# modelscope/FunASR

Hardware: AMD Instinct MI355X
Metric: audio-seconds/sec (RTF^-1) Paraformer-large 30s@bs64 (higher is better)
Workload: dtype f32 (GEMM / self-attention operands split into 2 fp16 planes, 3 fp16 MFMA products, f32 accumulate; all else f32)

## Files before the change

### funasr_amd/csrc/gemm_f16x2.hip

```cpp
#include "common.h"
#include <cstdlib>
#include <type_traits>
#include "gemm_f16x2_epilogue.h"

namespace pf {

namespace {

typedef _Float16 f16x8 __attribute__((ext_vector_type(8)));

template <int WM, int WN, int WGM = 4, int KS_ = 32> struct Geo2 {
    static constexpr int NW = WGM * 2;
    static constexpr int BM = WGM * WM * 32, BN = 2 * WN * 32;
    static constexpr int KS = KS_, ROWB = 2 * KS, CPR = ROWB / 16, RPP = 1024 / ROWB;
    static constexpr int SWZ = CPR == 4 ? 2 : 3;
    static constexpr int A_PLANE_B = BM * ROWB, B_PLANE_B = BN * ROWB;
    static constexpr int STAGE_B = 2 * (A_PLANE_B + B_PLANE_B);
    static constexpr int NSTG = KS == 16 ? (WGM == 4 ? (163840 / STAGE_B > 6 ? 6 : 163840 / STAGE_B) : 3) : 2;
    static constexpr int NPIECE = STAGE_B / 1024;
    static constexpr int A_PIECES = 2 * BM / RPP;
    static constexpr int PPW = NPIECE / NW;
    static constexpr int ELD = WN * 32 + 4;
    static constexpr int SLAB_B = NW * 32 * ELD * 4;
    static constexpr int LDS_B = NSTG * STAGE_B > SLAB_B ? NSTG * STAGE_B : SLAB_B;
};
template <int N> __device__ __forceinline__ void glds_wait_but() { asm volatile("s_waitcnt vmcnt(%0)" ::"i"(N) : "memory"); }

template <int WM, int WN, int MODE, int OUT, int ABL, int SCHED, int WGM, int KS_>
__device__ __forceinline__ void gemm2_tile_body(Gemm2Args& p, const int m0, const int n0, const int nblk, unsigned char* smem) {
    typedef Geo2<WM, WN, WGM, KS_> G;
    constexpr int BM = G::BM, BN = G::BN, KS = G::KS, ROWB = G::ROWB, CPR = G::CPR, RPP = G::RPP, PPW = G::PPW;
    constexpr int STAGE_B = G::STAGE_B, A_PLANE_B = G::A_PLANE_B, B_PLANE_B = G::B_PLANE_B;
    const int tid = threadIdx.x;
    const int lane = tid & 63;
    const int wave = __builtin_amdgcn_readfirstlane(tid >> 6);
    const int wr = wave >> 1, wc = wave & 1;
    const int hh = lane >> 5, idx = lane & 31;

    const unsigned short* src[PPW];
    {
        const int prow = lane / CPR;
        const int chunk = (lane % CPR) ^ ((prow >> G::SWZ) & (CPR - 1));
#pragma unroll
        for (int i = 0; i < PPW; ++i) {
            const int q = wave + G::NW * i;
            if (q < G::A_PIECES) {
                int row = m0 + (q % (BM / RPP)) * RPP + prow;
                row = row < p.M ? row : p.M - 1;
                src[i] = p.A + (size_t)(q / (BM / RPP)) * p.a_plane + (size_t)row * p.lda + chunk * 8;
            } else {
                const int qq = q - G::A_PIECES;
                int col = n0 + (qq % (BN / RPP)) * RPP + prow;
                col = col < p.N ? col : p.N - 1;
                src[i] = p.W + (size_t)(qq / (BN / RPP)) * p.w_plane + (size_t)col * p.ldw + chunk * 8;
            }
        }
    }
    const unsigned lds0 = __builtin_amdgcn_readfirstlane(lds_addr_of(smem) + (unsigned)wave * 1024);
    const size_t a_step = p.a_kstep > 0 ? (size_t)p.a_kstep : (size_t)KS, w_step = p.w_kstep > 0 ? (size_t)p.w_kstep : (size_t)KS;
    auto piece = [&](int i, int buf, int kt) {
        if constexpr (ABL == 3) return;
        glds16(src[i] + kt * (i < G::A_PIECES / G::NW ? a_step : w_step), lds0 + (unsigned)buf * STAGE_B + (unsigned)i * (G::NW * 1024));
    };

    floatx16 acc[WM][WN];
#pragma unroll
    for (int i = 0; i < WM; ++i)
#pragma unroll
        for (int jj = 0; jj < WN; ++jj)
#pragma unroll
            for (int r = 0; r < 16; ++r) acc[i][jj][r] = 0.f;

    const int f = (idx >> G::SWZ) & (CPR - 1);
    const int aoff = (wr * (WM * 32) + idx) * ROWB;
    const int boff = 2 * A_PLANE_B + (wc * (WN * 32) + idx) * ROWB;
    int coff[2];
#pragma unroll
    for (int st = 0; st < 2; ++st) coff[st] = ((2 * st + hh) ^ f) * 16;

    const int nk = p.K / KS;
    if constexpr (SCHED == 3) { if (wave >= 4) __builtin_amdgcn_s_setprio(1); }
    if constexpr (KS_ == 16 && WGM == 4) {
        constexpr int R = G::NSTG;
        static_assert(R == 5 && G::NPIECE == 32 && G::A_PIECES == 16 && RPP == 32, "deep ring: five 32-KB stages of 32-row pieces");
        const int grp = wave >> 1, hw = wave & 1;
        const int prow = lane / CPR;
        const unsigned chunkb = (unsigned)(((lane % CPR) ^ ((prow >> G::SWZ) & (CPR - 1))) * 16);
        const unsigned ldsb = __builtin_amdgcn_readfirstlane(lds_addr_of(smem));
        const size_t a_step2 = (p.a_kstep > 0 ? (size_t)p.a_kstep : (size_t)KS) * 2, w_step2 = (p.w_kstep > 0 ? (size_t)p.w_kstep : (size_t)KS) * 2;
        auto issue = [&](int kt, int buf, int i) {
            if constexpr (ABL == 3) return;
            const unsigned dst = ldsb + (unsigned)buf * STAGE_B + (unsigned)(hw + 2 * i) * 1024;
            if (i < 8) {
                int row = m0 + (hw + 2 * (i & 3)) * RPP + prow;
                row = row < p.M ? row : p.M - 1;
                glds16s(reinterpret_cast<const char*>(p.A) + (size_t)(i >> 2) * p.a_plane * 2 + (size_t)kt * a_step2,
                        (unsigned)row * (unsigned)p.lda * 2u + chunkb, dst);
            } else {
                int col = n0 + (hw + 2 * (i & 3)) * RPP + prow;
                col = col < p.N ? col : p.N - 1;
                glds16s(reinterpret_cast<const char*>(p.W) + (size_t)((i - 8) >> 2) * p.w_plane * 2 + (size_t)kt * w_step2,
                        (unsigned)col * (unsigned)p.ldw * 2u + chunkb, dst);
            }
        };
        auto issue_stage = [&](int kt, int buf) {
#pragma unroll
            for (int i = 0; i < 16; ++i) issue(kt, buf, i);
        };
        auto frags = [&](f16x8 (&a)[WM][2], f16x8 (&b)[WN][2], int buf) {
            const unsigned char* sb = smem + buf * STAGE_B;
#pragma unroll
            for (int pl = 1; pl >= 0; --pl) {
#pragma unroll
                for (int i = 0; i < WM; ++i)
                    a[i][pl] = __builtin_bit_cast(f16x8, *reinterpret_cast<const uint4*>(sb + pl * A_PLANE_B + aoff + i * 32 * ROWB + coff[0]));
            }
#pragma unroll
            for (int pl = 0; pl < 2; ++pl) {
#pragma unroll
                for (int jj = 0; jj < WN; ++jj)
                    b[jj][pl] = __builtin_bit_cast(f16x8, *reinterpret_cast<const uint4*>(sb + pl * B_PLANE_B + boff + jj * 32 * ROWB + coff[0]));
            }
        };
        if (grp < nk) issue_stage(grp, grp);
        if (grp == 0) glds_wait_all();
        __syncthreads();
        if (grp == 0 && 4 < nk) issue_stage(4, 4);
        f16x8 a0[WM][2], b0[WN][2], a1[WM][2], b1[WN][2];
        frags(a0, b0, 0);
        int buf = 0;
        auto step = [&](auto more, int kt, f16x8 (&a)[WM][2], f16x8 (&b)[WN][2], f16x8 (&an)[WM][2], f16x8 (&bn)[WN][2]) {
            const int nbuf = buf + 1 == R ? 0 : buf + 1;
            if constexpr (decltype(more)::value) {
                const bool own = grp == ((kt + 1) & 3);
                asm volatile("s_waitcnt lgkmcnt(0)" ::: "memory");
                if (own) glds_wait_all();
                __syncthreads();
                frags(an, bn, nbuf);
                if (own && kt + R < nk) issue_stage(kt + R, buf);
                __builtin_amdgcn_sched_barrier(0);
            }
#pragma unroll
            for (int i = 0; i < WM; ++i)
#pragma unroll
                for (int jj = 0; jj < WN; ++jj) acc[i][jj] = __builtin_amdgcn_mfma_f32_32x32x16_f16(a[i][1], b[jj][0], acc[i][jj], 0, 0, 0);
#pragma unroll
            for (int i = 0; i < WM; ++i)
#pragma unroll
                for (int jj = 0; jj < WN; ++jj) acc[i][jj] = __builtin_amdgcn_mfma_f32_32x32x16_f16(a[i][0], b[jj][1], acc[i][jj], 0, 0, 0);
#pragma unroll
            for (int i = 0; i < WM; ++i)
#pragma unroll
                for (int jj = 0; jj < WN; ++jj) acc[i][jj] = __builtin_amdgcn_mfma_f32_32x32x16_f16(a[i][0], b[jj][0], acc[i][jj], 0, 0, 0);
            buf = nbuf;
        };
        typedef std::integral_constant<bool, true> More;
        typedef std::integral_constant<bool, false> Last;
        for (int kt = 0; kt + 2 < nk; kt += 2) {
            step(More{}, kt, a0, b0, a1, b1);
            step(More{}, kt + 1, a1, b1, a0, b0);
        }
        step(More{}, nk - 2, a0, b0, a1, b1);
        step(Last{}, nk - 1, a1, b1, a0, b0);
    } else if constexpr (KS_ == 16) {
#pragma unroll
        for (int i = 0; i < PPW; ++i) piece(i, 0, 0);
        if (nk > 1) {
#pragma unroll
            for (int i = 0; i < PPW; ++i) piece(i, 1, 1);
        }
        for (int kt = 0; kt < nk; ++kt) {
            if (kt + 1 < nk) glds_wait_but<PPW>(); else glds_wait_all();
            __syncthreads();
            const unsigned char* sb = smem + (kt % 3) * STAGE_B;
            f16x8 a[WM][2], b[WN][2];
#pragma unroll
            for (int pl = 0; pl < 2; ++pl) {
#pragma unroll
                for (int i = 0; i < WM; ++i)
                    a[i][pl] = __builtin_bit_cast(f16x8, *reinterpret_cast<const uint4*>(sb + pl * A_PLANE_B + aoff + i * 32 * ROWB + coff[0]));
#pragma unroll
                for (int jj = 0; jj < WN; ++jj)
                    b[jj][pl] = __builtin_bit_cast(f16x8, *reinterpret_cast<const uint4*>(sb + pl * B_PLANE_B + boff + jj * 32 * ROWB + coff[0]));
            }
            if (kt + 2 < nk) {
#pragma unroll
                for (int i = 0; i < PPW; ++i) piece(i, (kt + 2) % 3, kt + 2);
            }
#define PF_PROD16(PA, PB)                                                                                             \
    _Pragma("unroll") for (int i = 0; i < WM; ++i) _Pragma("unroll") for (int jj = 0; jj < WN; ++jj)                  \
        acc[i][jj] = __builtin_amdgcn_mfma_f32_32x32x16_f16(a[i][PA], b[jj][PB], acc[i][jj], 0, 0, 0)
            PF_PROD16(1, 0);
            PF_PROD16(0, 1);
            PF_PROD16(0, 0);
#undef PF_PROD16
        }
    } else {
#pragma unroll
    for (int i = 0; i < PPW; ++i) piece(i, 0, 0);
    for (int kt = 0; kt < nk; ++kt) {
        glds_wait_all();
        __syncthreads();
        const bool nxt = kt + 1 < nk;
        const int nb = (kt + 1) & 1;
        const unsigned char* sb = smem + (kt & 1) * STAGE_B;
#define PF_PIECE(I) do { if ((I) < PPW && nxt) piece((I) < PPW ? (I) : 0, nb, kt + 1); } while (0)
#define PF_PROD(PA, PB)                                                                                               \
    _Pragma("unroll") for (int i = 0; i < WM; ++i) _Pragma("unroll") for (int jj = 0; jj < WN; ++jj)                  \
        acc[i][jj] = __builtin_amdgcn_mfma_f32_32x32x16_f16(a[i][PA], b[jj][PB], acc[i][jj], 0, 0, 0)
#define PF_LOAD(S)                                                                                                    \
    _Pragma("unroll") for (int pl = 0; pl < 2; ++pl) {                                                                \
        _Pragma("unroll") for (int i = 0; i < WM; ++i)                                                                \
            a[i][pl] = __builtin_bit_cast(f16x8, *reinterpret_cast<const uint4*>(sb + pl * A_PLANE_B + aoff + i * 32 * ROWB + coff[S]));   \
        _Pragma("unroll") for (int jj = 0; jj < WN; ++jj)                                                             \
            b[jj][pl] = __builtin_bit_cast(f16x8, *reinterpret_cast<const uint4*>(sb + pl * B_PLANE_B + boff + jj * 32 * ROWB + coff[S])); \
    }
        if constexpr (SCHED == 0 || SCHED == 3) {
            f16x8 a[WM][2], b[WN][2];
            PF_LOAD(0)
            PF_PROD(1, 0); PF_PIECE(0); PF_PIECE(1);
            PF_PROD(0, 1); PF_PIECE(2); PF_PIECE(3);
            PF_PROD(0, 0); PF_PIECE(4);
            PF_LOAD(1)
            PF_PROD(1, 0); PF_PIECE(5); PF_PIECE(6);
            PF_PROD(0, 1); PF_PIECE(7);
            PF_PROD(0, 0);
        } else {
            f16x8 a[WM][2], b[WN][2], a1[WM][2], b1[WN][2];
            PF_LOAD(0)
            {
#define a a1
#define b b1
                PF_LOAD(1)
#undef a
#undef b
            }
            if constexpr (SCHED == 2) { PF_PIECE(0); PF_PIECE(1); PF_PIECE(2); PF_PIECE(3); }
            PF_PROD(1, 0); if constexpr (SCHED == 1) { PF_PIECE(0); PF_PIECE(1); } else { PF_PIECE(4); PF_PIECE(5); }
            PF_PROD(0, 1); if constexpr (SCHED == 1) { PF_PIECE(2); PF_PIECE(3); } else { PF_PIECE(6); PF_PIECE(7); }
            PF_PROD(0, 0); if constexpr (SCHED == 1) { PF_PIECE(4); }
#define a a1
#define b b1
            PF_PROD(1, 0); if constexpr (SCHED == 1) { PF_PIECE(5); PF_PIECE(6); }
            PF_PROD(0, 1); if constexpr (SCHED == 1) { PF_PIECE(7); }
            PF_PROD(0, 0);
#undef a
#undef b
        }
#undef PF_PROD
#undef PF_LOAD
#undef PF_PIECE
    }
    }

    gemm2_epilogue<WM, WN, G::NW, MODE, OUT, ABL>(p, acc, smem, m0, n0, nblk, wave, wr, wc, lane);
}
template <int WM, int WN, int MODE, int OUT, int ABL = 0, int SCHED = 0, int WGM = 4, int KS_ = 32>
__global__ __launch_bounds__(WGM * 128, 2) void gemm_f16x2_kernel(Gemm2Args p, int nM, int nN) {
    typedef Geo2<WM, WN, WGM, KS_> G;
    constexpr int BM = G::BM, BN = G::BN;
    extern __shared__ __attribute__((aligned(16))) unsigned char smem[];

    const int L = blockIdx.x;
    const int xcd = L & 7, j8 = L >> 3;
    const int mblk = (j8 / nN) * 8 + xcd, nblk = j8 % nN;
    if (mblk >= nM) return;
    const int m0 = mblk * BM, n0 = nblk * BN;
    if constexpr (OUT == 0 && MODE == 0) {
        if (p.kslices > 1) {
            const size_t z = blockIdx.y;
            p.A += z * (size_t)p.K;
            p.W += z * (size_t)p.K;
            p.C += z * (size_t)p.M * (size_t)p.ldc;
        }
    }

    gemm2_tile_body<WM, WN, MODE, OUT, ABL, SCHED, WGM, KS_>(p, m0, n0, nblk, smem);
}


__global__ __launch_bounds__(256) void split2_kernel(const float* __restrict__ x, int ldx, unsigned short* __restrict__ y,
                                                     int ldy, size_t plane, int M, int N, float scale,
                                                     const float* __restrict__ scale_dev, int seq_out, int seq_in) {
    if (scale_dev) scale *= *scale_dev;
    const int c4n = ldy >> 2;
    const size_t total = (size_t)M * c4n;
    const bool wide_st = ldy % 8 == 0 && plane % 8 == 0 && ((uintptr_t)y & 15) == 0;
    for (size_t i = (size_t)blockIdx.x * 256 + threadIdx.x; i < total; i += (size_t)gridDim.x * 256) {
        const int row = (int)(i / c4n), c = (int)(i % c4n) * 4;
        int xrow = row;
        bool pad = false;
        if (seq_out > 0) {
            const int b = row / seq_out, t = row % seq_out;
            pad = t >= seq_in;
            xrow = b * seq_in + t;
        }
        float v[4] = {0.f, 0.f, 0.f, 0.f};
        if (pad) {
        } else if (c + 3 < N) {
            const float4 t = *reinterpret_cast<const float4*>(x + (size_t)xrow * ldx + c);
            v[0] = t.x; v[1] = t.y; v[2] = t.z; v[3] = t.w;
        } else {
#pragma unroll
            for (int e = 0; e < 4; ++e) if (c + e < N) v[e] = x[(size_t)xrow * ldx + c + e];
        }
        if (wide_st) store_split2x4_pair(y + (size_t)row * ldy + c, plane, v, scale, threadIdx.x);
        else store_split2x4(y + (size_t)row * ldy + c, plane, v, scale);
    }
}

__global__ __launch_bounds__(256) void absmax_kernel(const float* __restrict__ x, size_t n, unsigned* __restrict__ out) {
    float m = 0.f;
    for (size_t i = (size_t)blockIdx.x * 256 + threadIdx.x; i < n; i += (size_t)gridDim.x * 256) m = fmaxf(m, fabsf(x[i]));
    m = wave_max(m);
    if ((threadIdx.x & 63) == 0) atomicMax(out, __builtin_bit_cast(unsigned, m));
}

__global__ __launch_bounds__(256) void rowl1_bound_kernel(const float* __restrict__ W, int rows, int cols, int ld,
                                                          const float* __restrict__ bias, float in_bound, unsigned* __restrict__ out) {
    const int row = blockIdx.x * 4 + (threadIdx.x >> 6), lane = threadIdx.x & 63;
    if (row >= rows) return;
    float a = 0.f;
    for (int k = lane; k < cols; k += 64) a += fabsf(W[(size_t)row * ld + k]);
    a = wave_sum(a);
    const float bnd = (in_bound * a) * 1.0001f + (bias ? fabsf(bias[row]) : 0.f);
    if (lane == 0) atomicMax(out, __builtin_bit_cast(unsigned, bnd));
}

__global__ __launch_bounds__(256) void splitk_reduce_kernel(const float* __restrict__ part, int slices, size_t slice_stride, int M, int N,
                                                            const float* __restrict__ bias, int relu, const float* R1, int ldr1,
                                                            const float* R2, int ldr2, float* C, int ldc, unsigned short* C2, int ldc2,
                                                            size_t c_plane, float cscale) {
    const int n4 = N >> 2;
    const size_t total = (size_t)M * n4;
    for (size_t i = (size_t)blockIdx.x * 256 + threadIdx.x; i < total; i += (size_t)gridDim.x * 256) {
        const int row = (int)(i / n4), col = (int)(i % n4) * 4;
        const float* src = part + (size_t)row * N + col;
        float4 v = *reinterpret_cast<const float4*>(src);
        for (int z = 1; z < slices; ++z) {
            const float4 t = *reinterpret_cast<const float4*>(src + (size_t)z * slice_stride);
            v.x += t.x; v.y += t.y; v.z += t.z; v.w += t.w;
        }
        if (bias) {
            const float4 b = *reinterpret_cast<const float4*>(bias + col);
            v.x += b.x; v.y += b.y; v.z += b.z; v.w += b.w;
        }
        if (relu) { v.x = fmaxf(v.x, 0.f); v.y = fmaxf(v.y, 0.f); v.z = fmaxf(v.z, 0.f); v.w = fmaxf(v.w, 0.f); }
        if (R1) {
            const float4 r = *reinterpret_cast<const float4*>(R1 + (size_t)row * ldr1 + col);
            v.x = v.x + r.x; v.y = v.y + r.y; v.z = v.z + r.z; v.w = v.w + r.w;
        }
        if (R2) {
            const float4 r = *reinterpret_cast<const float4*>(R2 + (size_t)row * ldr2 + col);
            v.x = r.x + v.x; v.y = r.y + v.y; v.z = r.z + v.z; v.w = r.w + v.w;
        }
        if (C2) {
            const float o[4] = {v.x, v.y, v.z, v.w};
            store_split2x4(C2 + (size_t)row * ldc2 + col, c_plane, o, cscale);
        } else {
            *reinterpret_cast<float4*>(C + (size_t)row * ldc + col) = v;
        }
    }
}

template <int WM, int WN, int MODE, int OUT, int ABL = 0, int SCHED = 0, int WGM = 4, int KS_ = 32>
int launch_tile(const Gemm2Args& a, hipStream_t stream) {
    typedef Geo2<WM, WN, WGM, KS_> G;
    static PerDeviceOnce configured;
    if (!configured.done()) {
        PF_HIP_TRY(hipFuncSetAttribute(reinterpret_cast<const void*>(&gemm_f16x2_kernel<WM, WN, MODE, OUT, ABL, SCHED, WGM, KS_>),
                                       hipFuncAttributeMaxDynamicSharedMemorySize, G::LDS_B));
        configured.mark();
    }
    const int nM = ceil_div(a.M, G::BM), nN = ceil_div(a.N, G::BN);
    const int nMpad = (nM + 7) / 8 * 8;
    const unsigned gy = (OUT == 0 && MODE == 0 && a.kslices > 1) ? (unsigned)a.kslices : 1u;
    hipLaunchKernelGGL((gemm_f16x2_kernel<WM, WN, MODE, OUT, ABL, SCHED, WGM, KS_>), dim3((unsigned)nMpad * nN, gy), dim3(WGM * 128), G::LDS_B, stream, a, nM, nN);
    PF_HIP_TRY(hipGetLastError());
    return 0;
}
#if defined(PF_MEASUREMENT_KERNELS)
template <int MODE, int OUT>
int launch_pair(const Gemm2Args& a, hipStream_t stream) { return launch_tile<2, 4, MODE, OUT, 0, 0, 2, 16>(a, stream); }
template <int MODE, int OUT>
int launch_ring(const Gemm2Args& a, hipStream_t stream) { return launch_tile<2, 4, MODE, OUT, 0, 0, 4, 16>(a, stream); }
#endif
template <int MODE, int OUT>
int launch_one(const Gemm2Args& a, hipStream_t stream) {
    if constexpr (OUT == 1) {
        if (a.tile == 3) return launch_tile<2, 2, MODE, 1, 0, 0, 2>(a, stream);
    }
    if constexpr (OUT == 0) {
        if (a.tile == 3) return launch_tile<2, 2, MODE, 0, 0, 0, 2>(a, stream);
    }
#if defined(PF_MEASUREMENT_KERNELS)
    if constexpr (OUT == 0) {
        if (a.tile >= 256) return (a.tile >> 8) == 1 ? launch_tile<2, 4, MODE, 0, 0, 1>(a, stream) : launch_tile<2, 4, MODE, 0, 0, 2>(a, stream);
    }
    if constexpr (MODE == 0 && OUT == 0) {
        if (a.tile == 0x82) return launch_tile<2, 2, 0, 0, 2, 0, 2>(a, stream);
        if (a.tile == 0x83) return launch_tile<2, 2, 0, 0, 3, 0, 2>(a, stream);
        if (a.tile >= 16) {
            switch (a.tile >> 4) {
                case 1: return launch_tile<2, 4, 0, 0, 1>(a, stream);
                case 2: return launch_tile<2, 4, 0, 0, 2>(a, stream);
                case 3: return launch_tile<2, 4, 0, 0, 3>(a, stream);
                default: return launch_tile<2, 4, 0, 0, 4>(a, stream);
            }
        }
    }
#endif
    const int n_cu = device_cu_count();
    const long m_tiles = ceil_div(a.M, 256);
    const long wide_blocks = m_tiles * (a.N / 256), narrow_blocks = m_tiles * ceil_div(a.N, 128);
    const double cost_wide = (double)((wide_blocks + n_cu - 1) / n_cu), cost_narrow = 0.57 * (double)((narrow_blocks + n_cu - 1) / n_cu);
    const bool wide = a.tile == 2 || a.tile == 8 || a.tile == 9 || (a.tile == 0 && a.N % 256 == 0 && cost_wide <= cost_narrow);
    if constexpr (OUT == 0) {
        const long small_blocks = (long)ceil_div(a.M, 128) * ceil_div(a.N, 128);
        const double cost_small = 0.55 * (double)((small_blocks + 2 * n_cu - 1) / (2 * n_cu));
        if (a.tile == 0 && cost_small < (wide ? cost_wide : cost_narrow)) return launch_tile<2, 2, MODE, 0, 0, 0, 2>(a, stream);
    }
    if constexpr (OUT == 1) {
        if (a.tile == 0 && 2 * narrow_blocks <= n_cu) return launch_tile<2, 2, MODE, 1, 0, 0, 2>(a, stream);
    }
#if defined(PF_MEASUREMENT_KERNELS)
    if (wide && a.tile == 8) return launch_tile<2, 4, MODE, OUT, 0, 2>(a, stream);
    if (wide && a.tile == 9) return launch_tile<2, 4, MODE, OUT, 0, 3>(a, stream);
#endif
    return wide ? launch_tile<2, 4, MODE, OUT, 0, 0>(a, stream) : launch_tile<2, 2, MODE, OUT>(a, stream);
}

}

__global__ void pow2_scale_kernel(const float* __restrict__ amax, float* __restrict__ sc) {
    const float a = *amax;
    int e = a > 0.f ? (int)floorf(log2f(32768.f / a)) : 0;
    e = e > 100 ? 100 : (e < -100 ? -100 : e);
    sc[0] = ldexpf(1.f, e);
    sc[1] = ldexpf(1.f, -e);
}

int launch_pow2_scale(const float* amax_dev, float* sc, hipStream_t stream) {
    hipLaunchKernelGGL(pow2_scale_kernel, dim3(1), dim3(1), 0, stream, amax_dev, sc);
    PF_HIP_TRY(hipGetLastError());
    return 0;
}

__global__ void kv_scales_kernel(const float* __restrict__ amax, const float* __restrict__ lb, int n, float* __restrict__ out) {
    const int i = blockIdx.x * 64 + threadIdx.x;
    if (i >= 2 * n) return;
    const float bound = *amax * lb[2 * i] + lb[2 * i + 1];
    int e = bound > 0.f ? (int)floorf(log2f(32768.f / bound)) : 0;
    e = e > 60 ? 60 : (e < -60 ? -60 : e);
    out[4 * (i >> 1) + (i & 1)] = ldexpf(1.f, e);
    out[4 * (i >> 1) + 2 + (i & 1)] = ldexpf(1.f, -e);
}

int launch_kv_scales(const float* amax_dev, const float* l1_bmax_dev, int n_layers, float* out, hipStream_t stream) {
    hipLaunchKernelGGL(kv_scales_kernel, dim3(ceil_div(2 * n_layers, 64)), dim3(64), 0, stream, amax_dev, l1_bmax_dev, n_layers, out);
    PF_HIP_TRY(hipGetLastError());
    return 0;
}

int launch_split2(const float* x, int ldx, unsigned short* y, int ldy, size_t plane, int M, int N, float scale,
                  hipStream_t stream, const float* scale_dev, int seq_out, int seq_in) {
    PF_REQUIRE(M > 0 && N > 0 && ldy >= N && ldy % 4 == 0, "split2: ldy must cover N and be a multiple of 4");
    PF_REQUIRE(ldx % 4 == 0 && ((uintptr_t)x & 15) == 0 && ((uintptr_t)y & 7) == 0 && plane % 4 == 0, "split2: alignment");
    const size_t total = (size_t)M * (ldy >> 2);
    const unsigned blocks = (unsigned)((total + 255) / 256 < 8192 ? (total + 255) / 256 : 8192);
    hipLaunchKernelGGL(split2_kernel, dim3(blocks), dim3(256), 0, stream, x, ldx, y, ldy, plane, M, N, scale, scale_dev, seq_out, seq_in);
    PF_HIP_TRY(hipGetLastError());
    return 0;
}

int launch_absmax(const float* x, size_t n, float* out_dev, hipStream_t stream) {
    PF_HIP_TRY(hipMemsetAsync(out_dev, 0, sizeof(float), stream));
    const unsigned blocks = (unsigned)((n + 255) / 256 < 2048 ? (n + 255) / 256 : 2048);
    hipLaunchKernelGGL(absmax_kernel, dim3(blocks ? blocks : 1), dim3(256), 0, stream, x, n, reinterpret_cast<unsigned*>(out_dev));
    PF_HIP_TRY(hipGetLastError());
    return 0;
}

int launch_rowl1_bound(const float* W, int rows, int cols, int ld, const float* bias, float in_bound, float* out_dev,
                       hipStream_t stream) {
    PF_HIP_TRY(hipMemsetAsync(out_dev, 0, sizeof(float), stream));
    hipLaunchKernelGGL(rowl1_bound_kernel, dim3(ceil_div(rows, 4)), dim3(256), 0, stream, W, rows, cols, ld, bias, in_bound,
                       reinterpret_cast<unsigned*>(out_dev));
    PF_HIP_TRY(hipGetLastError());
    return 0;
}

static bool qkv_form_prefers_ps(const Gemm2Args& a) {
    static const int mode = [] { const char* e = getenv("PF_QKV_PS"); return e ? atoi(e) : 2; }();
    if (mode == 0 || !gemm_f16x2_ps_ok(a)) return false;
    if (mode == 1) return true;
    const int n_cu = device_cu_count();
    const long blocks = (long)ceil_div(a.M, 256) * (a.N / 256);
    if (blocks < n_cu) return false;
    const double rounds = (double)blocks / n_cu, whole = (double)((blocks + n_cu - 1) / n_cu);
    return whole / rounds > 1.15;
}

int gemm_f16x2_argmax_parts(int M, int N) { (void)M; return 2 * ceil_div(N, 256); }

int launch_gemm_f16x2(const Gemm2Args& a, hipStream_t stream) {
    PF_REQUIRE(a.M > 0 && a.N > 0 && a.K > 0, "gemm_f16x2: empty problem");
    if (a.ksplit > 1) {
        PF_REQUIRE((a.C || a.C2 || a.ln_g) && a.part && !a.amax_val && a.qkv_D <= 0 && a.a_kstep <= 0 && a.w_kstep <= 0 &&
                   a.K % (32 * a.ksplit) == 0 && a.N % 4 == 0 && ((uintptr_t)a.part & 15) == 0,
                   "gemm_f16x2: the split-K form needs K % (32 ksplit) == 0 and a partial buffer [ksplit][M][N]");
        if (a.C2) PF_REQUIRE(!a.ln_g && a.ldc2 % 4 == 0 && a.c_plane % 4 == 0 && ((uintptr_t)a.C2 & 7) == 0, "gemm_f16x2: split-K plane output alignment");
        else PF_REQUIRE((a.ln_g && !a.C) || (a.ldc % 4 == 0 && ((uintptr_t)a.C & 15) == 0), "gemm_f16x2: split-K output alignment");
        PF_REQUIRE(a.lda % 8 == 0 && a.ldw % 8 == 0 && a.a_plane % 8 == 0 && a.w_plane % 8 == 0 && ((uintptr_t)a.A & 15) == 0 &&
                   ((uintptr_t)a.W & 15) == 0 && (a.K / a.ksplit) % 8 == 0, "gemm_f16x2: operand alignment");
        if (a.bias) PF_REQUIRE(((uintptr_t)a.bias & 15) == 0, "gemm_f16x2: bias alignment");
        if (a.R1) PF_REQUIRE(a.ldr1 % 4 == 0 && ((uintptr_t)a.R1 & 15) == 0, "gemm_f16x2: R1 alignment");
        if (a.R2) PF_REQUIRE(a.ldr2 % 4 == 0 && ((uintptr_t)a.R2 & 15) == 0, "gemm_f16x2: R2 alignment");
        Gemm2Args p = a;
        p.ksplit = 0; p.kslices = a.ksplit; p.K = a.K / a.ksplit;
        p.C = a.part; p.ldc = a.N; p.C2 = nullptr; p.bias = nullptr; p.relu = 0; p.R1 = nullptr; p.R2 = nullptr; p.tile = 0;
        int rc = launch_tile<2, 2, 0, 0, 0, 0, 2>(p, stream);
        if (rc) return rc;
        if (a.ln_g) {
            PF_REQUIRE(a.ln_b && a.ln_y, "gemm_f16x2: the split-K + LayerNorm form needs beta and an output");
            return launch_splitk_reduce_ln(a.part, a.ksplit, (size_t)a.M * a.N, a.M, a.N, a.bias, a.relu, a.R1, a.ldr1, a.R2, a.ldr2, a.C, a.ldc, a.ln_g, a.ln_b,
                                           a.ln_eps, a.ln_y, a.ln_ldy, a.ln_out, a.ln_plane, a.ln_oscale, stream);
        }
        const size_t total = (size_t)a.M * (a.N >> 2);
        const unsigned blocks = (unsigned)((total + 255) / 256 < 4096 ? (total + 255) / 256 : 4096);
        hipLaunchKernelGGL(splitk_reduce_kernel, dim3(blocks), dim3(256), 0, stream, a.part, a.ksplit, (size_t)a.M * a.N, a.M, a.N,
                           a.bias, a.relu, a.R1, a.ldr1, a.R2, a.ldr2, a.C, a.ldc, a.C2, a.ldc2, a.c_plane, a.cscale);
        PF_HIP_TRY(hipGetLastError());
        return 0;
    }
    if (a.amax_val) {
        PF_REQUIRE(a.amax_idx && a.amax_ld >= gemm_f16x2_argmax_parts(a.M, a.N) && !a.R1 && !a.R2 && !a.relu && a.qkv_D <= 0,
                   "gemm_f16x2: the arg-max form takes bias only and needs amax_ld >= 2 ceil(N / 256)");
        PF_REQUIRE(a.K % 32 == 0 && a.lda % 8 == 0 && a.ldw % 8 == 0 && ((uintptr_t)a.A & 15) == 0 && ((uintptr_t)a.W & 15) == 0,
                   "gemm_f16x2: operand alignment");
        return launch_tile<2, 4, 0, 3, 0, 0>(a, stream);
    }
    PF_REQUIRE(a.K % 32 == 0, "gemm_f16x2: K must be a multiple of 32 (pad the planes with zeros)");
    PF_REQUIRE(a.lda % 8 == 0 && a.ldw % 8 == 0 && a.a_plane % 8 == 0 && a.w_plane % 8 == 0, "gemm_f16x2: operand strides % 8");
    PF_REQUIRE(((uintptr_t)a.A & 15) == 0 && ((uintptr_t)a.W & 15) == 0, "gemm_f16x2: operands must be 16-B aligned");
    PF_REQUIRE(a.N % 4 == 0, "gemm_f16x2: N % 4");
    if (a.C2 && a.qkv_D <= 0) PF_REQUIRE(a.ldc2 % 4 == 0 && a.c_plane % 4 == 0 && ((uintptr_t)a.C2 & 7) == 0, "gemm_f16x2: plane output alignment");
    else if (a.qkv_D <= 0 || a.C) PF_REQUIRE(a.C && a.ldc % 4 == 0 && ((uintptr_t)a.C & 15) == 0, "gemm_f16x2: output alignment");
    if (a.bias) PF_REQUIRE(((uintptr_t)a.bias & 15) == 0, "gemm_f16x2: bias alignment");
    if (a.R1) PF_REQUIRE(a.ldr1 % 4 == 0 && ((uintptr_t)a.R1 & 15) == 0, "gemm_f16x2: R1 alignment");
    if (a.R2) PF_REQUIRE(a.ldr2 % 4 == 0 && ((uintptr_t)a.R2 & 15) == 0, "gemm_f16x2: R2 alignment");
    const int mode = (a.R1 ? 1 : 0) | (a.R2 ? 2 : 0);
    if (a.qkv_D > 0) {
        PF_REQUIRE(mode == 0 && !a.relu && a.N == (a.kv_form ? 2 : 3) * a.qkv_D && a.qkv_D % 256 == 0 && a.M % 16 == 0,
                   "gemm_f16x2: the QKV / KV form needs N == 3 D (2 D), D % 256 == 0, M % 16 == 0, no residuals");
        PF_REQUIRE((a.kv_form || (a.Qp && a.C)) && a.Kp && a.VT && a.ldvt % 8 == 0 && a.vt_plane % 8 == 0 && a.qk_plane % 8 == 0 &&
                   ((uintptr_t)a.Qp & 15) == 0 && ((uintptr_t)a.Kp & 15) == 0 && ((uintptr_t)a.VT & 15) == 0,
                   "gemm_f16x2: QKV outputs");
    }
    if ((a.tile & 15) == 10 || (a.tile & 15) == 12) {
        if (gemm_f16x2_ps_ok(a)) return launch_gemm_f16x2_ps(a, stream);
        Gemm2Args b = a;
        b.tile = 0;
        return launch_gemm_f16x2(b, stream);
    }
    if ((a.tile & 15) == 7) {
        if (gemm_f16x2_w4_ok(a)) return launch_gemm_f16x2_w4(a, a.tile >> 4, stream);
        Gemm2Args b = a;
        b.tile = 0;
        return launch_gemm_f16x2(b, stream);
    }
#if !defined(PF_MEASUREMENT_KERNELS)
    PF_REQUIRE(a.tile == 0 || a.tile == 1 || a.tile == 2 || a.tile == 3 || a.tile == 7 || (a.tile & 15) == 10,
               "gemm_f16x2: this tile id is a measurement shape (libparaformer_hip_measure.so, make measure)");
#endif
    if (a.qkv_D > 0) {
#if defined(PF_MEASUREMENT_KERNELS)
        if (a.tile == 5) return launch_pair<0, 2>(a, stream);
        if (a.tile == 6) return launch_ring<0, 2>(a, stream);
#endif
        if (a.tile == 3) return launch_tile<2, 2, 0, 2, 0, 0, 2>(a, stream);
        if (a.tile == 0 && qkv_form_prefers_ps(a)) return launch_gemm_f16x2_ps(a, stream);
        if (a.tile == 0) {
            const int n_cu = device_cu_count();
            const int nN = a.N / 256, m_tiles = ceil_div(a.M, 256);
            const long blocks = (long)m_tiles * nN, full = blocks / n_cu, rem = blocks % n_cu;
            const double cost_wide = (double)(full + (rem ? 1 : 0));
            const double r_small = (double)ceil_div(a.M, 128) * (a.N / 128) / (2.0 * n_cu);
            const double cost_small = 0.6 * (r_small > 1.0 ? r_small : 1.0);
            const int head_tiles = (int)(full * n_cu / nN);
            const int tail_rows = a.M - head_tiles * 256;
            double cost_split = 1e30;
            if (full >= 2 && rem > 0 && tail_rows > 0 && (long)ceil_div(tail_rows, 128) * (a.N / 128) <= 2L * n_cu) cost_split = (double)full + 0.65;
            if (cost_small < cost_wide && cost_small <= cost_split) return launch_tile<2, 2, 0, 2, 0, 0, 2>(a, stream);
            if (cost_split < cost_wide) {
                Gemm2Args h = a, t = a;
                const size_t r0 = (size_t)head_tiles * 256;
                h.M = (int)r0;
                t.M = tail_rows;
                t.A = a.A + r0 * a.lda;
                if (a.C) t.C = a.C + r0 * a.ldc;
                if (a.Qp) t.Qp = a.Qp + r0 * a.qkv_D;
                t.Kp = a.Kp + r0 * a.qkv_D;
                t.VT = a.VT + r0;
                const int rc = launch_tile<2, 4, 0, 2, 0, 0>(h, stream);
                return rc ? rc : launch_tile<2, 2, 0, 2, 0, 0, 2>(t, stream);
            }
        }
#if defined(PF_MEASUREMENT_KERNELS)
        if (a.tile == 8) return launch_tile<2, 4, 0, 2, 0, 2>(a, stream);
        if (a.tile == 9) return launch_tile<2, 4, 0, 2, 0, 3>(a, stream);
#endif
        return launch_tile<2, 4, 0, 2, 0, 0>(a, stream);
    }
    if (a.C2) {
        PF_REQUIRE(mode == 0, "gemm_f16x2: the plane output has no residual form");
#if defined(PF_MEASUREMENT_KERNELS)
        if (a.tile == 5 && a.N % 256 == 0) return launch_pair<0, 1>(a, stream);
        if (a.tile == 6 && a.N % 256 == 0) return launch_ring<0, 1>(a, stream);
#endif
        return launch_one<0, 1>(a, stream);
    }
#if defined(PF_MEASUREMENT_KERNELS)
    if (a.tile == 5 && a.N % 256 == 0) {
        switch (mode) {
            case 0: return launch_pair<0, 0>(a, stream);
            case 1: return launch_pair<1, 0>(a, stream);
            case 2: return launch_pair<2, 0>(a, stream);
            default: return launch_pair<3, 0>(a, stream);
        }
    }
    if (a.tile == 6 && a.N % 256 == 0) {
        switch (mode) {
            case 0: return launch_ring<0, 0>(a, stream);
            case 1: return launch_ring<1, 0>(a, stream);
            case 2: return launch_ring<2, 0>(a, stream);
            default: return launch_ring<3, 0>(a, stream);
        }
    }
#endif
    switch (mode) {
        case 0: return launch_one<0, 0>(a, stream);
        case 1: return launch_one<1, 0>(a, stream);
        case 2: return launch_one<2, 0>(a, stream);
        default: return launch_one<3, 0>(a, stream);
    }
}

}
```

### funasr_amd/csrc/gemm_f16x2_epilogue.h

```cpp
#pragma once
#include "common.h"

namespace pf {

template <int WM, int WN, int NW, int MODE, int OUT, int ABL>
__device__ __forceinline__ void gemm2_epilogue(const Gemm2Args& p, floatx16 (&acc)[WM][WN], unsigned char* smem, int m0, int n0, int nblk,
                                               int wave, int wr, int wc, int lane) {
    const int hh = lane >> 5, idx = lane & 31;
    constexpr int ELD_ = WN * 32 + 4;
    if constexpr (ABL == 2) {
        float t = 0.f;
#pragma unroll
        for (int i = 0; i < WM; ++i)
#pragma unroll
            for (int jj = 0; jj < WN; ++jj)
#pragma unroll
                for (int r = 0; r < 16; ++r) t += acc[i][jj][r];
        if (t == 123.456f) p.C[0] = t;
        return;
    }
    if constexpr (OUT == 3) {
        const float osc = p.oscale_dev ? p.oscale * *p.oscale_dev : p.oscale;
        float bv[WN];
#pragma unroll
        for (int jj = 0; jj < WN; ++jj) {
            const int col = n0 + wc * (WN * 32) + jj * 32 + idx;
            bv[jj] = (p.bias && col < p.N) ? p.bias[col] : 0.f;
        }
#pragma unroll
        for (int i = 0; i < WM; ++i) {
#pragma unroll
            for (int r = 0; r < 16; ++r) {
                const int row = m0 + wr * (WM * 32) + i * 32 + (r & 3) + 8 * (r >> 2) + 4 * hh;
                float best = -INFINITY;
                int besti = 0x7fffffff;
#pragma unroll
                for (int jj = 0; jj < WN; ++jj) {
                    const int col = n0 + wc * (WN * 32) + jj * 32 + idx;
                    if (col < p.N) {
                        const float v = acc[i][jj][r] * osc + bv[jj];
                        if (v > best) { best = v; besti = col; }
                    }
                }
#pragma unroll
                for (int o = 16; o > 0; o >>= 1) {
                    const float ov = __shfl_xor(best, o, 64);
                    const int oi = __shfl_xor(besti, o, 64);
                    if (ov > best || (ov == best && oi < besti)) { best = ov; besti = oi; }
                }
                if (idx == 0 && row < p.M) {
                    const size_t o = (size_t)row * p.amax_ld + 2 * nblk + wc;
                    p.amax_val[o] = best;
                    p.amax_idx[o] = besti;
                }
            }
        }
        return;
    }
    constexpr bool HAS_R1 = (MODE & 1) != 0, HAS_R2 = (MODE & 2) != 0;
    constexpr int ELD = ELD_;
    constexpr int LPR = WN * 8;
    constexpr int RPS = 64 / LPR;
    constexpr int NPASS = 32 / RPS;
    __syncthreads();
    float* slab = reinterpret_cast<float*>(smem) + wave * (32 * ELD);
    const int c4 = lane % LPR, rsub = lane / LPR;
    const int col = n0 + wc * (WN * 32) + c4 * 4;
    const bool colok = col + 3 < p.N;
    const bool wide_st = OUT == 1 && p.N % 8 == 0 && p.ldc2 % 8 == 0 && p.c_plane % 8 == 0 && ((uintptr_t)p.C2 & 15) == 0;
    const float oscale = p.oscale_dev ? p.oscale * *p.oscale_dev : p.oscale;
    float4 bias4 = make_float4(0.f, 0.f, 0.f, 0.f);
    if (p.bias && colok) bias4 = *reinterpret_cast<const float4*>(p.bias + col);
#pragma unroll
    for (int i = 0; i < WM; ++i) {
#pragma unroll
        for (int jj = 0; jj < WN; ++jj)
#pragma unroll
            for (int r = 0; r < 16; ++r)
                slab[((r & 3) + 8 * (r >> 2) + 4 * hh) * ELD + jj * 32 + idx] = acc[i][jj][r];
        const int row0 = m0 + wr * (WM * 32) + i * 32 + rsub;
        if (!colok) continue;
        const int seg = OUT == 2 ? n0 / p.qkv_D + (p.kv_form ? 1 : 0) : 0;
        const int scol = OUT == 2 ? col - (n0 / p.qkv_D) * p.qkv_D : col;
        float k_mul = p.k_mul, v_mul = p.v_mul;
        if constexpr (OUT == 2) {
            if (p.kv_mul_dev) { k_mul *= p.kv_mul_dev[0]; v_mul *= p.kv_mul_dev[1]; }
        }
#pragma unroll
        for (int h2 = 0; h2 < NPASS / 8; ++h2) {
            float4 v[8], r1[8], r2[8];
#pragma unroll
            for (int it = 0; it < 8; ++it)
                v[it] = *reinterpret_cast<const float4*>(slab + ((h2 * 8 + it) * RPS + rsub) * ELD + c4 * 4);
#pragma unroll
            for (int it = 0; it < 8; ++it) {
                const int row = row0 + (h2 * 8 + it) * RPS;
                const int rr = row < p.M ? row : p.M - 1;
                if constexpr (HAS_R1) r1[it] = *reinterpret_cast<const float4*>(p.R1 + (size_t)rr * p.ldr1 + col);
                if constexpr (HAS_R2) r2[it] = *reinterpret_cast<const float4*>(p.R2 + (size_t)rr * p.ldr2 + col);
            }
#pragma unroll
            for (int it = 0; it < 8; ++it) {
                const int row = row0 + (h2 * 8 + it) * RPS;
                float o[4] = {v[it].x * oscale + bias4.x, v[it].y * oscale + bias4.y, v[it].z * oscale + bias4.z,
                              v[it].w * oscale + bias4.w};
                if (p.relu) {
#pragma unroll
                    for (int e = 0; e < 4; ++e) o[e] = fmaxf(o[e], 0.f);
                }
                if constexpr (HAS_R1) { o[0] = o[0] + r1[it].x; o[1] = o[1] + r1[it].y; o[2] = o[2] + r1[it].z; o[3] = o[3] + r1[it].w; }
                if constexpr (HAS_R2) { o[0] = r2[it].x + o[0]; o[1] = r2[it].y + o[1]; o[2] = r2[it].z + o[2]; o[3] = r2[it].w + o[3]; }
                if (row >= p.M) continue;
                if constexpr (ABL == 1) { if (o[0] == 123.456f) p.C[0] = o[1] + o[2] + o[3]; continue; }
                if constexpr (OUT == 2) {
                    if (seg == 0) store_split2x4_pair(p.Qp + (size_t)row * p.qkv_D + scol, p.qk_plane, o, p.q_mul, lane);
                    else if (seg == 1) store_split2x4_pair(p.Kp + (size_t)row * p.qkv_D + scol, p.qk_plane, o, k_mul, lane);
                    else if (p.C) *reinterpret_cast<float4*>(p.C + (size_t)row * p.ldc + scol) = make_float4(o[0], o[1], o[2], o[3]);
                } else if constexpr (OUT == 1) {
                    if (wide_st) store_split2x4_pair(p.C2 + (size_t)row * p.ldc2 + col, p.c_plane, o, p.cscale, lane);
                    else store_split2x4(p.C2 + (size_t)row * p.ldc2 + col, p.c_plane, o, p.cscale);
                } else if constexpr (ABL == 4) {
                    *reinterpret_cast<float4*>(p.C + (size_t)(row & 63) * 256 + (col & 255)) = make_float4(o[0], o[1], o[2], o[3]);
                } else {
                    *reinterpret_cast<float4*>(p.C + (size_t)row * p.ldc + col) = make_float4(o[0], o[1], o[2], o[3]);
                }
            }
        }
        if constexpr (OUT == 2) {
            if (seg == 2) {
                const int vc0 = n0 - (p.kv_form ? 1 : 2) * p.qkv_D + wc * (WN * 32);
#pragma unroll
                for (int ps = 0; ps < WN * 32 * 4 / 64; ++ps) {
                    const int piece = ps * 64 + lane;
                    const int nl = piece >> 2, G = (piece >> 1) & 1, half = piece & 1;
                    const int rb = 16 * G + 4 * half;
                    const float bv = p.bias ? p.bias[n0 + wc * (WN * 32) + nl] : 0.f;
                    float t[8];
#pragma unroll
                    for (int j = 0; j < 8; ++j)
                        t[j] = (slab[(rb + (j & 3) + 8 * (j >> 2)) * ELD + nl] * oscale + bv) * v_mul;
                    const int mb = m0 + wr * (WM * 32) + i * 32 + 16 * G;
                    if (mb < p.M) {
                        uint4 h, l;
                        split2_pk(t[0], t[1], h.x, l.x);
                        split2_pk(t[2], t[3], h.y, l.y);
                        split2_pk(t[4], t[5], h.z, l.z);
                        split2_pk(t[6], t[7], h.w, l.w);
                        unsigned short* vp = p.VT + (size_t)(vc0 + nl) * p.ldvt + mb + 8 * half;
                        *reinterpret_cast<uint4*>(vp) = h;
                        *reinterpret_cast<uint4*>(vp + p.vt_plane) = l;
                    }
                }
            }
        }
    }
}

}
```

### funasr_amd/csrc/gemm_f16x2_row.hip

```cpp
#include "common.h"
#include "gemm_f16x2_row_epilogue.h"

namespace pf {

namespace {

typedef _Float16 f16x8 __attribute__((ext_vector_type(8)));


template <int MODE, bool LN, bool A_NT, int SCHED = 2>
__global__ __launch_bounds__(512, 2) void gemm_f16x2_row_kernel(GemmRowArgs p) {
    constexpr int WM = 2, WN = 4;
    extern __shared__ __attribute__((aligned(16))) unsigned char smem[];

    const int m0 = blockIdx.x * RW_BM;
    const int tid = threadIdx.x;
    const int lane = tid & 63;
    const int wave = __builtin_amdgcn_readfirstlane(tid >> 6);
    const int wr = wave >> 2, wc = wave & 3;
    const int hh = lane >> 5, idx = lane & 31;

    const unsigned short* src[RW_PPW];
    {
        const int prow = lane >> 2;
        const int chunk = (lane & 3) ^ ((prow >> 2) & 3);
        int row = m0 + wave * 16 + prow;
        row = row < p.M ? row : p.M - 1;
        src[0] = p.A + (size_t)row * p.lda + chunk * 8;
        src[1] = src[0] + p.a_plane;
#pragma unroll
        for (int j = 0; j < 4; ++j) {
            const int col = (wave + 8 * j) * 16 + prow;
            src[2 + j] = p.W + (size_t)col * p.ldw + chunk * 8;
            src[6 + j] = src[2 + j] + p.w_plane;
        }
    }
    const unsigned lds0 = __builtin_amdgcn_readfirstlane(lds_addr_of(smem) + (unsigned)wave * 1024);
    auto piece = [&](int i, int buf, int kt) {
        const unsigned dst = lds0 + (unsigned)buf * RW_STAGE_B + (unsigned)i * 8192;
        if (A_NT && i < 2) glds16_nt(src[i] + kt * RW_KS, dst);
        else glds16(src[i] + kt * RW_KS, dst);
    };

    floatx16 acc[WM][WN];
#pragma unroll
    for (int i = 0; i < WM; ++i)
#pragma unroll
        for (int jj = 0; jj < WN; ++jj)
#pragma unroll
            for (int r = 0; r < 16; ++r) acc[i][jj][r] = 0.f;

    const int f = (idx >> 2) & 3;
    const int aoff = (wr * 64 + idx) * RW_ROWB;
    const int boff = 2 * RW_A_PLANE_B + (wc * 128 + idx) * RW_ROWB;
    int coff[2];
#pragma unroll
    for (int st = 0; st < 2; ++st) coff[st] = ((2 * st + hh) ^ f) * 16;

#if defined(PF_MEASUREMENT_KERNELS)
    const int nk = (p.a_nt & 128) ? 0 : p.K / RW_KS;
#else
    const int nk = p.K / RW_KS;
#endif
    constexpr int PF_R2_LINES = RW_BM * 16, PF_V_LINES = (RW_BM + RW_FS_KS - 1) * 16;
#if defined(PF_MEASUREMENT_KERNELS)
    const bool pf_on = (MODE & 4) && (p.a_nt & 12) && nk > 1;
#else
    constexpr bool pf_on = false;
#endif
    const int pf_first = (p.a_nt & 4) ? 0 : PF_R2_LINES, pf_last = (p.a_nt & 8) ? PF_R2_LINES + PF_V_LINES : PF_R2_LINES;
    const int pf_per_stage = pf_on ? (pf_last - pf_first + nk - 2) / (nk - 1) : 0;
    unsigned pf_sink = 0;
    if (nk > 0) {
#pragma unroll
        for (int i = 0; i < RW_PPW; ++i) piece(i, 0, 0);
    }
    for (int kt = 0; kt < nk; ++kt) {
        glds_wait_all();
        asm volatile("" : : "v"(pf_sink));
        __syncthreads();
        if (pf_on && kt + 1 < nk) {
            for (int l = tid; l < pf_per_stage; l += 512) {
                const int idx = pf_first + kt * pf_per_stage + l;
                const float* src_line = nullptr;
                if (idx >= pf_last) {
                } else if (idx < PF_R2_LINES) {
                    int row = m0 + (idx >> 4);
                    row = row < p.M ? row : p.M - 1;
                    src_line = p.R2 + (size_t)row * p.ldr2 + (idx & 15) * 32;
                } else if (idx < PF_R2_LINES + PF_V_LINES) {
                    const int j = idx - PF_R2_LINES;
                    int row = m0 - RW_FS_LP + (j >> 4);
                    row = row < 0 ? 0 : (row < p.M ? row : p.M - 1);
                    src_line = p.fs_v + (size_t)row * p.ldfv + (j & 15) * 32;
                }
                if (src_line) asm volatile("global_load_dword %0, %1, off" : "=v"(pf_sink) : "v"(src_line) : "memory");
            }
        }
        const bool nxt = kt + 1 < nk;
        const int nb = (kt + 1) & 1;
        const unsigned char* sb = smem + (kt & 1) * RW_STAGE_B;
#if defined(PF_MEASUREMENT_KERNELS)
        const bool early = (p.a_nt & 512) != 0;
        if (early && nxt) {
#pragma unroll
            for (int i = 0; i < RW_PPW; ++i) piece(i, nb, kt + 1);
        }
#else
        constexpr bool early = false;
#endif
#define RW_PIECE(I) do { if (nxt && !early) piece(I, nb, kt + 1); } while (0)
#define RW_PROD(AF, BF, PA, PB)                                                                                       \
    _Pragma("unroll") for (int i = 0; i < WM; ++i) _Pragma("unroll") for (int jj = 0; jj < WN; ++jj)                  \
        acc[i][jj] = __builtin_amdgcn_mfma_f32_32x32x16_f16(AF[i][PA], BF[jj][PB], acc[i][jj], 0, 0, 0)
#define RW_LOAD(AF, BF, S)                                                                                            \
    _Pragma("unroll") for (int pl = 0; pl < 2; ++pl) {                                                                \
        _Pragma("unroll") for (int i = 0; i < WM; ++i)                                                                \
            AF[i][pl] = __builtin_bit_cast(f16x8, *reinterpret_cast<const uint4*>(sb + pl * RW_A_PLANE_B + aoff + i * 32 * RW_ROWB + coff[S]));   \
        _Pragma("unroll") for (int jj = 0; jj < WN; ++jj)                                                             \
            BF[jj][pl] = __builtin_bit_cast(f16x8, *reinterpret_cast<const uint4*>(sb + pl * RW_B_PLANE_B + boff + jj * 32 * RW_ROWB + coff[S])); \
    }
        f16x8 a0[WM][2], b0[WN][2], a1[WM][2], b1[WN][2];
        if constexpr (SCHED == 2) {
            RW_LOAD(a0, b0, 0)
            RW_LOAD(a1, b1, 1)
            RW_PIECE(0); RW_PIECE(1); RW_PIECE(2); RW_PIECE(3);
            RW_PROD(a0, b0, 1, 0); RW_PIECE(4); RW_PIECE(5);
            RW_PROD(a0, b0, 0, 1); RW_PIECE(6); RW_PIECE(7);
            RW_PROD(a0, b0, 0, 0); RW_PIECE(8); RW_PIECE(9);
            RW_PROD(a1, b1, 1, 0);
            RW_PROD(a1, b1, 0, 1);
            RW_PROD(a1, b1, 0, 0);
        } else {
            RW_LOAD(a0, b0, 0)
            RW_PROD(a0, b0, 1, 0); RW_PIECE(0); RW_PIECE(1); RW_PIECE(2);
            RW_PROD(a0, b0, 0, 1); RW_PIECE(3); RW_PIECE(4); RW_PIECE(5);
            RW_PROD(a0, b0, 0, 0); RW_PIECE(6); RW_PIECE(7);
            RW_LOAD(a1, b1, 1)
            RW_PROD(a1, b1, 1, 0); RW_PIECE(8); RW_PIECE(9);
            RW_PROD(a1, b1, 0, 1);
            RW_PROD(a1, b1, 0, 0);
        }
#undef RW_PROD
#undef RW_LOAD
#undef RW_PIECE
    }
#if defined(PF_MEASUREMENT_KERNELS)
    if (p.a_nt & 256) {
        float sacc = 0.f;
#pragma unroll
        for (int i = 0; i < WM; ++i)
#pragma unroll
            for (int jj = 0; jj < WN; ++jj)
#pragma unroll
                for (int r = 0; r < 16; ++r) sacc += acc[i][jj][r];
        if (sacc == 12345.678f && p.C) p.C[tid] = sacc;
        return;
    }
#endif
    if (pf_on) {
        glds_wait_all();
        asm volatile("" : : "v"(pf_sink));
    }

    gemm2_row_epilogue<MODE, LN, 512, WM, 0>(p, acc, smem, m0, tid, wave, wr, wc, lane, true);
}

template <int MODE, bool LN, bool A_NT, int SCHED = 2>
int launch_row_t(const GemmRowArgs& a, hipStream_t stream) {
    static PerDeviceOnce configured;
    if (!configured.done()) {
        PF_HIP_TRY(hipFuncSetAttribute(reinterpret_cast<const void*>(&gemm_f16x2_row_kernel<MODE, LN, A_NT, SCHED>),
                                       hipFuncAttributeMaxDynamicSharedMemorySize, RW_LDS_B));
        configured.mark();
    }
    hipLaunchKernelGGL((gemm_f16x2_row_kernel<MODE, LN, A_NT, SCHED>), dim3((unsigned)ceil_div(a.M, RW_BM)), dim3(512), RW_LDS_B, stream, a);
    PF_HIP_TRY(hipGetLastError());
    return 0;
}
template <int MODE, bool LN>
int launch_row_m(const GemmRowArgs& a, hipStream_t stream) {
#if defined(PF_MEASUREMENT_KERNELS)
    if (!(a.a_nt & 2)) return (a.a_nt & 1) ? launch_row_t<MODE, LN, true>(a, stream) : launch_row_t<MODE, LN, false>(a, stream);
#endif
    return (a.a_nt & 1) ? launch_row_t<MODE, LN, true, 0>(a, stream) : launch_row_t<MODE, LN, false, 0>(a, stream);
}

}

bool gemm_f16x2_row_applicable(int N, int K) { return N == RW_BN && K > 0 && K % RW_KS == 0; }

int launch_gemm_f16x2_row(const GemmRowArgs& a, hipStream_t stream) {
    PF_REQUIRE(a.M > 0 && a.N == RW_BN && a.K > 0 && a.K % RW_KS == 0, "gemm_f16x2_row: N must be 512 and K a multiple of 32");
    PF_REQUIRE(a.lda % 8 == 0 && a.ldw % 8 == 0 && a.a_plane % 8 == 0 && a.w_plane % 8 == 0, "gemm_f16x2_row: operand strides % 8");
    PF_REQUIRE(((uintptr_t)a.A & 15) == 0 && ((uintptr_t)a.W & 15) == 0, "gemm_f16x2_row: operands must be 16-B aligned");
    if (a.C) PF_REQUIRE(a.ldc % 4 == 0 && ((uintptr_t)a.C & 15) == 0, "gemm_f16x2_row: C alignment");
    if (a.bias) PF_REQUIRE(((uintptr_t)a.bias & 15) == 0, "gemm_f16x2_row: bias alignment");
    if (a.R1) PF_REQUIRE(a.ldr1 % 4 == 0 && ((uintptr_t)a.R1 & 15) == 0, "gemm_f16x2_row: R1 alignment");
    if (a.R2) PF_REQUIRE(a.ldr2 % 4 == 0 && ((uintptr_t)a.R2 & 15) == 0, "gemm_f16x2_row: R2 alignment");
    const bool ln = a.ln_g != nullptr;
    if (ln) {
        PF_REQUIRE(a.ln_b && ((uintptr_t)a.ln_g & 15) == 0 && ((uintptr_t)a.ln_b & 15) == 0, "gemm_f16x2_row: LayerNorm parameters");
        PF_REQUIRE((a.Y2 != nullptr) != (a.Yf != nullptr), "gemm_f16x2_row: the LayerNorm form writes planes (Y2) or fp32 (Yf)");
        if (a.Y2) PF_REQUIRE(a.ldy2 % 8 == 0 && a.y_plane % 8 == 0 && ((uintptr_t)a.Y2 & 15) == 0, "gemm_f16x2_row: plane output alignment");
        else PF_REQUIRE(a.ldyf % 4 == 0 && ((uintptr_t)a.Yf & 15) == 0, "gemm_f16x2_row: fp32 LayerNorm output alignment");
    } else {
        PF_REQUIRE(a.C, "gemm_f16x2_row: nothing to write");
    }
    if (a.fs_v)
        PF_REQUIRE(!a.R1 && a.fs_w && a.fs_lo && a.fs_hi && a.ldfv % 4 == 0 && ((uintptr_t)a.fs_v & 15) == 0 && a.M % 16 == 0 && ln,
                   "gemm_f16x2_row: the FSMN form needs taps, the 16-row group bounds, M % 16 == 0, the LayerNorm epilogue and no R1");
#if defined(PF_MEASUREMENT_KERNELS)
    static const int env_prefetch = [] { const char* e = getenv("PF_ROW_PREFETCH"); return e ? atoi(e) : -1; }();
    const int env_bits = (env_prefetch & ~3) | ((env_prefetch & 3) == 1 ? 12 : (env_prefetch & 3) == 2 ? 4 : (env_prefetch & 3) == 3 ? 8 : 0);
    if (env_prefetch >= 0 && a.fs_v && a.R2 && (a.a_nt & ~3) != env_bits) {
        GemmRowArgs b = a;
        b.a_nt = (a.a_nt & 3) | env_bits;
        return launch_gemm_f16x2_row(b, stream);
    }
#endif
    int bm = a.block_rows;
    if (bm == 0) {
        const int n_cu = device_cu_count();
        const double cost128 = (double)ceil_div(ceil_div(a.M, 128), n_cu), cost96 = 0.80 * (double)ceil_div(ceil_div(a.M, 96), n_cu);
        bm = cost96 < cost128 - 0.02 ? 96 : 128;
    }
#if defined(PF_MEASUREMENT_KERNELS)
    if (bm == 130) return launch_gemm_f16x2_w4_row(a, stream);
    if (bm != 128) {
        PF_REQUIRE(bm == 96 || bm == 129, "gemm_f16x2_row: block_rows is 0, 96, 128, 129 or 130");
#else
    if (bm != 128) {
        PF_REQUIRE(bm == 96, "gemm_f16x2_row: block_rows is 0, 96 or 128 (129 / 130: the measurement library, make measure)");
#endif
        const int rc = launch_gemm_f16x2_row8(a, bm == 96 ? 96 : 128, stream);
        if (rc != -3) return rc;
    }
    if (a.fs_v) return a.R2 ? launch_row_m<6, true>(a, stream) : launch_row_m<4, true>(a, stream);
    const int mode = (a.R1 ? 1 : 0) | (a.R2 ? 2 : 0);
    switch (mode * 2 + (ln ? 1 : 0)) {
        case 0: return launch_row_m<0, false>(a, stream);
        case 1: return launch_row_m<0, true>(a, stream);
        case 2: return launch_row_m<1, false>(a, stream);
        case 3: return launch_row_m<1, true>(a, stream);
        case 4: return launch_row_m<2, false>(a, stream);
        case 5: return launch_row_m<2, true>(a, stream);
        case 6: return launch_row_m<3, false>(a, stream);
        default: return launch_row_m<3, true>(a, stream);
    }
}

}
```

### funasr_amd/csrc/gemm_f16x2_row8.hip

```cpp
#include "common.h"

namespace pf {

namespace {

typedef _Float16 f16x8 __attribute__((ext_vector_type(8)));

constexpr int R8_BN = 512, R8_KS = 32, R8_ROWB = 64;
constexpr int R8_B_PLANE_B = R8_BN * R8_ROWB;
constexpr int R8_ELD = 132;
constexpr int R8_SLAB_B = 4 * 32 * R8_ELD * 4;
constexpr int R8_FS_KS = 11, R8_FS_LP = 5;
constexpr int R8_FSW_OFF_B = R8_SLAB_B;

template <int WM> struct R8Geo {
    static constexpr int BM = 32 * WM;
    static constexpr int A_PLANE_B = BM * R8_ROWB;
    static constexpr int STAGE_B = 2 * (A_PLANE_B + R8_B_PLANE_B);
    static constexpr int LDS_B = 2 * STAGE_B;
    static constexpr int NA = 4 * WM;
    static constexpr int P_FLOATS = BM * 128;
    static_assert(LDS_B <= 163840, "two stages must fit the CU's LDS");
    static_assert(R8_FSW_OFF_B + R8_FS_KS * R8_BN * 4 <= LDS_B && (P_FLOATS + 2 * BM) * 4 <= LDS_B, "epilogue LDS");
    static_assert(NA > 8 && NA <= 16, "a wave carries one or two A pieces");
};

template <int WM, int MODE, bool LN, bool A_NT>
__global__ __launch_bounds__(512, 2) void gemm_f16x2_row8_kernel(GemmRowArgs p) {
    typedef R8Geo<WM> G;
    constexpr int BM = G::BM, A_PLANE_B = G::A_PLANE_B, STAGE_B = G::STAGE_B, NA = G::NA;
    extern __shared__ __attribute__((aligned(16))) unsigned char smem[];

    const int m0 = blockIdx.x * BM;
    const int tid = threadIdx.x;
    const int lane = tid & 63;
    const int wave = __builtin_amdgcn_readfirstlane(tid >> 6);
    const int pc = wave >> 1, q = wave & 1;
    const int hh = lane >> 5, idx = lane & 31;

    const bool has_a1 = wave + 8 < NA;
    const unsigned short* src_a[2];
    const unsigned short* src_w[8];
    {
        const int prow = lane >> 2;
        const int chunk = (lane & 3) ^ ((prow >> 2) & 3);
#pragma unroll
        for (int j = 0; j < 2; ++j) {
            const int a = (wave + 8 * j) < NA ? wave + 8 * j : wave;
            int row = m0 + (a % (2 * WM)) * 16 + prow;
            row = row < p.M ? row : p.M - 1;
            src_a[j] = p.A + (size_t)(a / (2 * WM)) * p.a_plane + (size_t)row * p.lda + chunk * 8;
        }
#pragma unroll
        for (int j = 0; j < 8; ++j) {
            const int v = wave + 8 * j;
            const int col = (v & 31) * 16 + prow;
            src_w[j] = p.W + (size_t)(v >> 5) * p.w_plane + (size_t)col * p.ldw + chunk * 8;
        }
    }
    const unsigned lds0 = __builtin_amdgcn_readfirstlane(lds_addr_of(smem));
    auto piece_a = [&](int j, int buf, int kt) {
        const unsigned dst = lds0 + (unsigned)buf * STAGE_B + (unsigned)(wave + 8 * j) * 1024;
        if (A_NT) glds16_nt(src_a[j] + kt * R8_KS, dst);
        else glds16(src_a[j] + kt * R8_KS, dst);
    };
    auto piece_w = [&](int j, int buf, int kt) {
        glds16(src_w[j] + kt * R8_KS, lds0 + (unsigned)buf * STAGE_B + 2 * A_PLANE_B + (unsigned)(wave + 8 * j) * 1024);
    };

    floatx16 acc[WM][2];
#pragma unroll
    for (int i = 0; i < WM; ++i)
#pragma unroll
        for (int jj = 0; jj < 2; ++jj)
#pragma unroll
            for (int r = 0; r < 16; ++r) acc[i][jj][r] = 0.f;

    const int f = (idx >> 2) & 3;
    const int aoff = idx * R8_ROWB;
    const int boff = 2 * A_PLANE_B + (wave * 64 + idx) * R8_ROWB;
    int coff[2];
#pragma unroll
    for (int st = 0; st < 2; ++st) coff[st] = ((2 * st + hh) ^ f) * 16;

    const int nk = p.K / R8_KS;
    piece_a(0, 0, 0);
    if (has_a1) piece_a(1, 0, 0);
#pragma unroll
    for (int j = 0; j < 8; ++j) piece_w(j, 0, 0);
    for (int kt = 0; kt < nk; ++kt) {
        glds_wait_all();
        __syncthreads();
        const bool nxt = kt + 1 < nk;
        const int nb = (kt + 1) & 1;
        const unsigned char* sb = smem + (kt & 1) * STAGE_B;
#define R8_PROD(AF, BF, PA, PB)                                                                                       \
    _Pragma("unroll") for (int i = 0; i < WM; ++i) _Pragma("unroll") for (int jj = 0; jj < 2; ++jj)                   \
        acc[i][jj] = __builtin_amdgcn_mfma_f32_32x32x16_f16(AF[i][PA], BF[jj][PB], acc[i][jj], 0, 0, 0)
#define R8_LOAD(AF, BF, S)                                                                                            \
    _Pragma("unroll") for (int pl = 0; pl < 2; ++pl) {                                                                \
        _Pragma("unroll") for (int i = 0; i < WM; ++i)                                                                \
            AF[i][pl] = __builtin_bit_cast(f16x8, *reinterpret_cast<const uint4*>(sb + pl * A_PLANE_B + aoff + i * 32 * R8_ROWB + coff[S]));     \
        _Pragma("unroll") for (int jj = 0; jj < 2; ++jj)                                                              \
            BF[jj][pl] = __builtin_bit_cast(f16x8, *reinterpret_cast<const uint4*>(sb + pl * R8_B_PLANE_B + boff + jj * 32 * R8_ROWB + coff[S])); \
    }
        f16x8 a0[WM][2], b0[2][2], a1[WM][2], b1[2][2];
        R8_LOAD(a0, b0, 0)
        R8_LOAD(a1, b1, 1)
        if (nxt) { piece_a(0, nb, kt + 1); if (has_a1) piece_a(1, nb, kt + 1); piece_w(0, nb, kt + 1); piece_w(1, nb, kt + 1); }
        R8_PROD(a0, b0, 1, 0); if (nxt) { piece_w(2, nb, kt + 1); piece_w(3, nb, kt + 1); }
        R8_PROD(a0, b0, 0, 1); if (nxt) { piece_w(4, nb, kt + 1); piece_w(5, nb, kt + 1); }
        R8_PROD(a0, b0, 0, 0); if (nxt) { piece_w(6, nb, kt + 1); piece_w(7, nb, kt + 1); }
        R8_PROD(a1, b1, 1, 0);
        R8_PROD(a1, b1, 0, 1);
        R8_PROD(a1, b1, 0, 0);
#undef R8_PROD
#undef R8_LOAD
    }

    constexpr bool HAS_R1 = (MODE & 1) != 0, HAS_R2 = (MODE & 2) != 0, FSMN = (MODE & 4) != 0;
    static_assert(!(HAS_R1 && FSMN), "the FSMN form computes the first addend");
    float* smf = reinterpret_cast<float*>(smem);
    float* slab = smf + pc * (32 * R8_ELD);
    const float* fsw = reinterpret_cast<const float*>(smem + R8_FSW_OFF_B);
    const int c4 = idx, rsub = hh;
    const int col = pc * 128 + c4 * 4;
    const float oscale = p.oscale_dev ? p.oscale * *p.oscale_dev : p.oscale;
    float4 bias4 = make_float4(0.f, 0.f, 0.f, 0.f);
    if (p.bias) bias4 = *reinterpret_cast<const float4*>(p.bias + col);
    float4 ov[WM][8];
#pragma unroll
    for (int i = 0; i < WM; ++i) {
        __syncthreads();
        if constexpr (FSMN) {
            if (i == 0) {
                float* dst = reinterpret_cast<float*>(smem + R8_FSW_OFF_B);
#pragma unroll
                for (int j = 0; j < R8_FS_KS; ++j) dst[j * R8_BN + tid] = p.fs_w[(size_t)tid * R8_FS_KS + j];
            }
        }
#pragma unroll
        for (int jj = 0; jj < 2; ++jj)
#pragma unroll
            for (int r = 0; r < 16; ++r)
                slab[((r & 3) + 8 * (r >> 2) + 4 * hh) * R8_ELD + q * 64 + jj * 32 + idx] = acc[i][jj][r];
        __syncthreads();
        const int rl0 = q * 16 + rsub * 8;
        const int row0 = m0 + i * 32 + rl0;
        if constexpr (FSMN) {
            const int grp = row0 >> 4;
            const bool gok = row0 < p.M;
            const int lo = gok ? p.fs_lo[grp] : 0, hi = gok ? p.fs_hi[grp] : 0;
            float4 win[8 + R8_FS_KS - 1];
            auto load_row = [&](int k) {
                const int vr = row0 - R8_FS_LP + k;
                const bool ok = vr >= lo && vr < hi;
                const float4 t = *reinterpret_cast<const float4*>(p.fs_v + (size_t)(ok ? vr : (lo < hi ? lo : 0)) * p.ldfv + col);
                win[k] = ok ? t : make_float4(0.f, 0.f, 0.f, 0.f);
            };
#pragma unroll
            for (int k = 0; k < R8_FS_KS - 1; ++k) load_row(k);
#pragma unroll
            for (int h4 = 0; h4 < 2; ++h4) {
                float4 r2[4], fa[4];
#pragma unroll
                for (int t = 0; t < 4; ++t) {
                    load_row(R8_FS_KS - 1 + h4 * 4 + t);
                    fa[t] = make_float4(0.f, 0.f, 0.f, 0.f);
                    if constexpr (HAS_R2) {
                        const int row = row0 + h4 * 4 + t;
                        r2[t] = *reinterpret_cast<const float4*>(p.R2 + (size_t)(row < p.M ? row : p.M - 1) * p.ldr2 + col);
                    }
                }
#pragma unroll
                for (int j = 0; j < R8_FS_KS; ++j) {
                    const float4 wj = *reinterpret_cast<const float4*>(fsw + j * R8_BN + col);
#pragma unroll
                    for (int t = 0; t < 4; ++t) {
                        const float4 x = win[h4 * 4 + t + j];
                        fa[t].x = fmaf(wj.x, x.x, fa[t].x); fa[t].y = fmaf(wj.y, x.y, fa[t].y);
                        fa[t].z = fmaf(wj.z, x.z, fa[t].z); fa[t].w = fmaf(wj.w, x.w, fa[t].w);
                    }
                }
#pragma unroll
                for (int t = 0; t < 4; ++t) {
                    const int row = row0 + h4 * 4 + t;
                    const float4 c = win[h4 * 4 + t + R8_FS_LP];
                    float4 mem = make_float4(0.f, 0.f, 0.f, 0.f);
                    if (row < hi) mem = make_float4(fa[t].x + c.x, fa[t].y + c.y, fa[t].z + c.z, fa[t].w + c.w);
                    const float4 vt = *reinterpret_cast<const float4*>(slab + (rl0 + h4 * 4 + t) * R8_ELD + c4 * 4);
                    float o[4] = {vt.x * oscale + bias4.x, vt.y * oscale + bias4.y, vt.z * oscale + bias4.z,
                                  vt.w * oscale + bias4.w};
                    if (p.relu) {
#pragma unroll
                        for (int e = 0; e < 4; ++e) o[e] = fmaxf(o[e], 0.f);
                    }
                    o[0] = o[0] + mem.x; o[1] = o[1] + mem.y; o[2] = o[2] + mem.z; o[3] = o[3] + mem.w;
                    if constexpr (HAS_R2) { o[0] = r2[t].x + o[0]; o[1] = r2[t].y + o[1]; o[2] = r2[t].z + o[2]; o[3] = r2[t].w + o[3]; }
                    const float4 o4 = make_float4(o[0], o[1], o[2], o[3]);
                    ov[i][h4 * 4 + t] = o4;
                    if (p.C && row < p.M) *reinterpret_cast<float4*>(p.C + (size_t)row * p.ldc + col) = o4;
                }
                __builtin_amdgcn_sched_barrier(0);
            }
        } else {
            float4 v[8], r1[8], r2[8];
#pragma unroll
            for (int t = 0; t < 8; ++t)
                v[t] = *reinterpret_cast<const float4*>(slab + (rl0 + t) * R8_ELD + c4 * 4);
#pragma unroll
            for (int t = 0; t < 8; ++t) {
                const int row = row0 + t;
                const int rr = row < p.M ? row : p.M - 1;
                if constexpr (HAS_R1) r1[t] = *reinterpret_cast<const float4*>(p.R1 + (size_t)rr * p.ldr1 + col);
                if constexpr (HAS_R2) r2[t] = *reinterpret_cast<const float4*>(p.R2 + (size_t)rr * p.ldr2 + col);
            }
#pragma unroll
            for (int t = 0; t < 8; ++t) {
                const int row = row0 + t;
                float o[4] = {v[t].x * oscale + bias4.x, v[t].y * oscale + bias4.y, v[t].z * oscale + bias4.z,
                              v[t].w * oscale + bias4.w};
                if (p.relu) {
#pragma unroll
                    for (int e = 0; e < 4; ++e) o[e] = fmaxf(o[e], 0.f);
                }
                if constexpr (HAS_R1) { o[0] = o[0] + r1[t].x; o[1] = o[1] + r1[t].y; o[2] = o[2] + r1[t].z; o[3] = o[3] + r1[t].w; }
                if constexpr (HAS_R2) { o[0] = r2[t].x + o[0]; o[1] = r2[t].y + o[1]; o[2] = r2[t].z + o[2]; o[3] = r2[t].w + o[3]; }
                const float4 o4 = make_float4(o[0], o[1], o[2], o[3]);
                ov[i][t] = o4;
                if (p.C && row < p.M) *reinterpret_cast<float4*>(p.C + (size_t)row * p.ldc + col) = o4;
            }
            __builtin_amdgcn_sched_barrier(0);
        }
    }
    if constexpr (!LN) return;

    float* P = smf;
    float* ST = smf + G::P_FLOATS;
    const int lrow0 = q * 16 + rsub * 8;
    auto reduce_rows = [&](bool second) {
#pragma unroll
        for (int j = 0; j < BM / 16; ++j) {
            const int rl = wave * (BM / 8) + rsub * (BM / 16) + j;
            const float* pr = P + (size_t)rl * 128 + c4;
            float v = (pr[0] + pr[64]) + (pr[32] + pr[96]);
#pragma unroll
            for (int o = 16; o > 0; o >>= 1) v += __shfl_xor(v, o, 64);
            const float res = second ? ln_rstd(v, R8_BN, p.ln_eps) : ln_mean(v, R8_BN);
            if (c4 == 0) ST[(second ? BM : 0) + rl] = res;
        }
    };
    __syncthreads();
#pragma unroll
    for (int i = 0; i < WM; ++i)
#pragma unroll
        for (int t = 0; t < 8; ++t)
            P[(size_t)(lrow0 + 32 * i + t) * 128 + pc * 32 + c4] = ln_sum4(ov[i][t]);
    __syncthreads();
    reduce_rows(false);
    __syncthreads();
#pragma unroll
    for (int i = 0; i < WM; ++i)
#pragma unroll
        for (int t = 0; t < 8; ++t) {
            const float mean = ST[lrow0 + 32 * i + t];
            P[(size_t)(lrow0 + 32 * i + t) * 128 + pc * 32 + c4] = ln_sqdev4(ov[i][t], mean);
        }
    __syncthreads();
    reduce_rows(true);
    __syncthreads();
    const float4 g4 = *reinterpret_cast<const float4*>(p.ln_g + col);
    const float4 b4 = *reinterpret_cast<const float4*>(p.ln_b + col);
#pragma unroll
    for (int i = 0; i < WM; ++i)
#pragma unroll
        for (int t = 0; t < 8; ++t) {
            const int rl = lrow0 + 32 * i + t;
            const int row = m0 + rl;
            if (row >= p.M) continue;
            const float4 y = ln_apply4(ov[i][t], ST[rl], ST[BM + rl], g4, b4);
            if (p.Y2) {
                const float yv[4] = {y.x, y.y, y.z, y.w};
                store_split2x4_pair(p.Y2 + (size_t)row * p.ldy2 + col, p.y_plane, yv, p.yscale, lane);
            } else {
                *reinterpret_cast<float4*>(p.Yf + (size_t)row * p.ldyf + col) = y;
            }
        }
}

template <int WM, int MODE, bool LN, bool A_NT>
int launch_row8_t(const GemmRowArgs& a, hipStream_t stream) {
    typedef R8Geo<WM> G;
    static PerDeviceOnce configured;
    if (!configured.done()) {
        PF_HIP_TRY(hipFuncSetAttribute(reinterpret_cast<const void*>(&gemm_f16x2_row8_kernel<WM, MODE, LN, A_NT>),
                                       hipFuncAttributeMaxDynamicSharedMemorySize, G::LDS_B));
        configured.mark();
    }
    hipLaunchKernelGGL((gemm_f16x2_row8_kernel<WM, MODE, LN, A_NT>), dim3((unsigned)ceil_div(a.M, G::BM)), dim3(512), G::LDS_B, stream, a);
    PF_HIP_TRY(hipGetLastError());
    return 0;
}
template <int WM, int MODE, bool LN>
int launch_row8_m(const GemmRowArgs& a, hipStream_t stream) {
    return (a.a_nt & 1) ? launch_row8_t<WM, MODE, LN, true>(a, stream) : launch_row8_t<WM, MODE, LN, false>(a, stream);
}
template <int WM>
int launch_row8_w(const GemmRowArgs& a, hipStream_t stream) {
    const bool ln = a.ln_g != nullptr;
    if (a.fs_v) return a.R2 ? launch_row8_m<WM, 6, true>(a, stream) : launch_row8_m<WM, 4, true>(a, stream);
    const int mode = (a.R1 ? 1 : 0) | (a.R2 ? 2 : 0);
    switch (mode * 2 + (ln ? 1 : 0)) {
        case 0: return launch_row8_m<WM, 0, false>(a, stream);
        case 1: return launch_row8_m<WM, 0, true>(a, stream);
        case 3: return launch_row8_m<WM, 1, true>(a, stream);
        case 4: return launch_row8_m<WM, 2, false>(a, stream);
        case 5: return launch_row8_m<WM, 2, true>(a, stream);
        case 7: return launch_row8_m<WM, 3, true>(a, stream);
        default: return -3;
    }
}

}

int launch_gemm_f16x2_row8(const GemmRowArgs& a, int bm, hipStream_t stream) {
    if (bm == 96) return launch_row8_w<3>(a, stream);
#if defined(PF_MEASUREMENT_KERNELS)
    if (bm == 128) return launch_row8_w<4>(a, stream);
#endif
    return -3;
}

}
```

### funasr_amd/csrc/gemm_f16x2_row_epilogue.h

```cpp
#pragma once
#include "common.h"

namespace pf {

constexpr int RW_BM = 128, RW_BN = 512, RW_KS = 32, RW_ROWB = 64;
constexpr int RW_A_PLANE_B = RW_BM * RW_ROWB;
constexpr int RW_B_PLANE_B = RW_BN * RW_ROWB;
constexpr int RW_STAGE_B = 2 * (RW_A_PLANE_B + RW_B_PLANE_B);
constexpr int RW_PPW = RW_STAGE_B / 1024 / 8;
constexpr int RW_ELD = 132;
constexpr int RW_SLAB_B = 8 * 32 * RW_ELD * 4;
constexpr int RW_LDS_B = 2 * RW_STAGE_B;
constexpr int RW_P_FLOATS = RW_BM * 4 * 32;
constexpr int RW_FS_KS = 11, RW_FS_LP = 5;
constexpr int RW_FSW_OFF_B = RW_SLAB_B;
static_assert(RW_SLAB_B <= RW_LDS_B && (RW_P_FLOATS + 2 * RW_BM) * 4 <= RW_LDS_B, "epilogue LDS");
static_assert(RW_FSW_OFF_B + RW_FS_KS * RW_BN * 4 <= RW_LDS_B, "FSMN taps do not fit behind the slabs");

template <int MODE, bool LN, int NT, int AM, int I0>
__device__ __forceinline__ void gemm2_row_epilogue(const GemmRowArgs& p, floatx16 (&accf)[AM][4], unsigned char* smem, int m0, int tid,
                                                   int wave, int wr, int wc, int lane, bool stage_taps) {
    constexpr int WM = 2, WN = 4;
    const int hh = lane >> 5, idx = lane & 31;
    floatx16 (&acc_)[AM][4] = accf;
#if defined(PF_MEASUREMENT_KERNELS)
    const int abl = p.a_nt;
#else
    constexpr int abl = 0;
#endif
#define acc(i, jj) acc_[I0 + (i)][jj]
    constexpr bool HAS_R1 = (MODE & 1) != 0, HAS_R2 = (MODE & 2) != 0, FSMN = (MODE & 4) != 0;
    static_assert(!(HAS_R1 && FSMN), "the FSMN form computes the first addend");
    __syncthreads();
    float* smf = reinterpret_cast<float*>(smem);
    float* slab = smf + wave * (32 * RW_ELD);
    const float* fsw = reinterpret_cast<const float*>(smem + RW_FSW_OFF_B);
    if constexpr (FSMN) {
        if (stage_taps) {
            float* dst = reinterpret_cast<float*>(smem + RW_FSW_OFF_B);
#pragma unroll
            for (int c = tid; c < RW_BN; c += NT)
#pragma unroll
                for (int j = 0; j < RW_FS_KS; ++j) dst[j * RW_BN + c] = p.fs_w[(size_t)c * RW_FS_KS + j];
        }
        __syncthreads();
    }
    const int c4 = idx, rsub = hh;
    const int col = wc * 128 + c4 * 4;
    const float oscale = p.oscale_dev ? p.oscale * *p.oscale_dev : p.oscale;
    float4 bias4 = make_float4(0.f, 0.f, 0.f, 0.f);
    if (p.bias) bias4 = *reinterpret_cast<const float4*>(p.bias + col);
    float4 ov[WM][16];
#pragma unroll
    for (int i = 0; i < WM; ++i) {
#pragma unroll
        for (int jj = 0; jj < WN; ++jj)
#pragma unroll
            for (int r = 0; r < 16; ++r)
                slab[((r & 3) + 8 * (r >> 2) + 4 * hh) * RW_ELD + jj * 32 + idx] = acc(i, jj)[r];
        const int row0 = m0 + wr * 64 + i * 32 + rsub * 16;
        if constexpr (FSMN) {
            const int grp = row0 >> 4;
            const bool gok = row0 < p.M;
            const int lo = gok ? p.fs_lo[grp] : 0, hi = gok ? p.fs_hi[grp] : 0;
            float4 win[16 + RW_FS_KS - 1];
            auto load_row = [&](int k) {
                const int vr = row0 - RW_FS_LP + k;
                const bool ok = vr >= lo && vr < hi;
                float4 t = make_float4(0.f, 0.f, 0.f, 0.f);
                if (!(abl & 16)) t = *reinterpret_cast<const float4*>(p.fs_v + (size_t)(ok ? vr : (lo < hi ? lo : 0)) * p.ldfv + col);
                win[k] = ok ? t : make_float4(0.f, 0.f, 0.f, 0.f);
            };
#pragma unroll
            for (int k = 0; k < RW_FS_KS - 1; ++k) load_row(k);
#pragma unroll
            for (int h4 = 0; h4 < 4; ++h4) {
                float4 r2[4], fa[4];
#pragma unroll
                for (int t = 0; t < 4; ++t) {
                    load_row(RW_FS_KS - 1 + h4 * 4 + t);
                    fa[t] = make_float4(0.f, 0.f, 0.f, 0.f);
                    if constexpr (HAS_R2) {
                        const int row = row0 + h4 * 4 + t;
                        r2[t] = make_float4(0.f, 0.f, 0.f, 0.f);
                        if (!(abl & 32)) r2[t] = *reinterpret_cast<const float4*>(p.R2 + (size_t)(row < p.M ? row : p.M - 1) * p.ldr2 + col);
                    }
                }
#pragma unroll
                for (int j = 0; j < RW_FS_KS; ++j) {
                    const float4 wj = *reinterpret_cast<const float4*>(fsw + j * RW_BN + col);
#pragma unroll
                    for (int t = 0; t < 4; ++t) {
                        const float4 x = win[h4 * 4 + t + j];
                        fa[t].x = fmaf(wj.x, x.x, fa[t].x); fa[t].y = fmaf(wj.y, x.y, fa[t].y);
                        fa[t].z = fmaf(wj.z, x.z, fa[t].z); fa[t].w = fmaf(wj.w, x.w, fa[t].w);
                    }
                }
#pragma unroll
                for (int t = 0; t < 4; ++t) {
                    const int row = row0 + h4 * 4 + t;
                    const float4 c = win[h4 * 4 + t + RW_FS_LP];
                    float4 mem = make_float4(0.f, 0.f, 0.f, 0.f);
                    if (row < hi) mem = make_float4(fa[t].x + c.x, fa[t].y + c.y, fa[t].z + c.z, fa[t].w + c.w);
                    const float4 vt = *reinterpret_cast<const float4*>(slab + (rsub * 16 + h4 * 4 + t) * RW_ELD + c4 * 4);
                    float o[4] = {vt.x * oscale + bias4.x, vt.y * oscale + bias4.y, vt.z * oscale + bias4.z,
                                  vt.w * oscale + bias4.w};
                    if (p.relu) {
#pragma unroll
                        for (int e = 0; e < 4; ++e) o[e] = fmaxf(o[e], 0.f);
                    }
                    o[0] = o[0] + mem.x; o[1] = o[1] + mem.y; o[2] = o[2] + mem.z; o[3] = o[3] + mem.w;
                    if constexpr (HAS_R2) { o[0] = r2[t].x + o[0]; o[1] = r2[t].y + o[1]; o[2] = r2[t].z + o[2]; o[3] = r2[t].w + o[3]; }
                    const float4 o4 = make_float4(o[0], o[1], o[2], o[3]);
                    ov[i][h4 * 4 + t] = o4;
                    if (p.C && row < p.M && !(abl & 64)) *reinterpret_cast<float4*>(p.C + (size_t)row * p.ldc + col) = o4;
                }
                __builtin_amdgcn_sched_barrier(0);
            }
            continue;
        }
#pragma unroll
        for (int h2 = 0; h2 < 2; ++h2) {
            float4 v[8], r1[8], r2[8];
#pragma unroll
            for (int t = 0; t < 8; ++t)
                v[t] = *reinterpret_cast<const float4*>(slab + (rsub * 16 + h2 * 8 + t) * RW_ELD + c4 * 4);
#pragma unroll
            for (int t = 0; t < 8; ++t) {
                const int row = row0 + h2 * 8 + t;
                const int rr = row < p.M ? row : p.M - 1;
                if constexpr (HAS_R1) r1[t] = *reinterpret_cast<const float4*>(p.R1 + (size_t)rr * p.ldr1 + col);
                if constexpr (HAS_R2) r2[t] = *reinterpret_cast<const float4*>(p.R2 + (size_t)rr * p.ldr2 + col);
            }
#pragma unroll
            for (int t = 0; t < 8; ++t) {
                const int row = row0 + h2 * 8 + t;
                float o[4] = {v[t].x * oscale + bias4.x, v[t].y * oscale + bias4.y, v[t].z * oscale + bias4.z,
                              v[t].w * oscale + bias4.w};
                if (p.relu) {
#pragma unroll
                    for (int e = 0; e < 4; ++e) o[e] = fmaxf(o[e], 0.f);
                }
                if constexpr (HAS_R1) { o[0] = o[0] + r1[t].x; o[1] = o[1] + r1[t].y; o[2] = o[2] + r1[t].z; o[3] = o[3] + r1[t].w; }
                if constexpr (HAS_R2) { o[0] = r2[t].x + o[0]; o[1] = r2[t].y + o[1]; o[2] = r2[t].z + o[2]; o[3] = r2[t].w + o[3]; }
                const float4 o4 = make_float4(o[0], o[1], o[2], o[3]);
                ov[i][h2 * 8 + t] = o4;
                if (p.C && row < p.M) *reinterpret_cast<float4*>(p.C + (size_t)row * p.ldc + col) = o4;
            }
            __builtin_amdgcn_sched_barrier(0);
        }
    }
    if constexpr (!LN) return;

    float* P = smf;
    float* ST = smf + RW_P_FLOATS;
    const int lrow0 = wr * 64 + rsub * 16;
    auto reduce_rows = [&](bool second) {
#pragma unroll
        for (int j = 0; j < 8; ++j) {
            const int rl = wr * 64 + wc * 16 + rsub * 8 + j;
            const float* pr = P + (size_t)rl * 128 + c4;
            float v = (pr[0] + pr[64]) + (pr[32] + pr[96]);
#pragma unroll
            for (int o = 16; o > 0; o >>= 1) v += __shfl_xor(v, o, 64);
            const float res = second ? ln_rstd(v, RW_BN, p.ln_eps) : ln_mean(v, RW_BN);
            if (c4 == 0) ST[(second ? RW_BM : 0) + rl] = res;
        }
    };
    __syncthreads();
#pragma unroll
    for (int i = 0; i < WM; ++i)
#pragma unroll
        for (int it = 0; it < 16; ++it)
            P[(size_t)(lrow0 + 32 * i + it) * 128 + wc * 32 + c4] = ln_sum4(ov[i][it]);
    __syncthreads();
    reduce_rows(false);
    __syncthreads();
#pragma unroll
    for (int i = 0; i < WM; ++i)
#pragma unroll
        for (int it = 0; it < 16; ++it) {
            const float mean = ST[lrow0 + 32 * i + it];
            P[(size_t)(lrow0 + 32 * i + it) * 128 + wc * 32 + c4] = ln_sqdev4(ov[i][it], mean);
        }
    __syncthreads();
    reduce_rows(true);
    __syncthreads();
    const float4 g4 = *reinterpret_cast<const float4*>(p.ln_g + col);
    const float4 b4 = *reinterpret_cast<const float4*>(p.ln_b + col);
#pragma unroll
    for (int i = 0; i < WM; ++i)
#pragma unroll
        for (int it = 0; it < 16; ++it) {
            const int rl = lrow0 + 32 * i + it;
            const int row = m0 + rl;
            if (row >= p.M || (abl & 64)) continue;
            const float4 y = ln_apply4(ov[i][it], ST[rl], ST[RW_BM + rl], g4, b4);
            if (p.Y2) {
                const float yv[4] = {y.x, y.y, y.z, y.w};
                store_split2x4_pair(p.Y2 + (size_t)row * p.ldy2 + col, p.y_plane, yv, p.yscale, lane);
            } else {
                *reinterpret_cast<float4*>(p.Yf + (size_t)row * p.ldyf + col) = y;
            }
        }
#undef acc
}

}
```

### funasr_amd/csrc/gemm_f16x2_w4.hip

```cpp
#include "common.h"
#include "gemm_f16x2_epilogue.h"
#include "gemm_f16x2_row_epilogue.h"

namespace pf {

namespace {

typedef _Float16 f16x8 __attribute__((ext_vector_type(8)));

template <int GM_, int GN_> struct W4Geo {
    static constexpr int GM = GM_, GN = GN_;
    static constexpr int BM = GM * 128, BN = GN * 128;
    static constexpr int A_PLANE_B = BM * 64, W_PLANE_B = BN * 64;
    static constexpr int STAGE_B = 2 * (A_PLANE_B + W_PLANE_B);
    static constexpr int NPW = STAGE_B / 1024 / 4;
    static constexpr int TA = BM / 64, TW = BN / 64;
    static constexpr int LDS_B = 2 * STAGE_B;
    static_assert(GM * GN == 4 && NPW == 2 * (TA + TW), "four waves");
};

struct W4Frags { f16x8 al[4], ah[4], bh[4], bl[4]; };

__device__ __forceinline__ void w4_mfma(floatx16& acc, const f16x8& a, const f16x8& b) {
    asm volatile("v_mfma_f32_32x32x16_f16 %0, %1, %2, %0" : "+a"(acc) : "v"(a), "v"(b));
}
template <int OFF> __device__ __forceinline__ void w4_read(f16x8& dst, unsigned addr) {
    asm volatile("ds_read_b128 %0, %1 offset:%2" : "=v"(dst) : "v"(addr), "n"(OFF));
}
__device__ __forceinline__ void w4_reads_done(W4Frags& f) {
    asm volatile("s_waitcnt lgkmcnt(0)"
                 : "+v"(f.al[0]), "+v"(f.al[1]), "+v"(f.al[2]), "+v"(f.al[3]), "+v"(f.ah[0]), "+v"(f.ah[1]), "+v"(f.ah[2]), "+v"(f.ah[3]),
                   "+v"(f.bh[0]), "+v"(f.bh[1]), "+v"(f.bh[2]), "+v"(f.bh[3]), "+v"(f.bl[0]), "+v"(f.bl[1]), "+v"(f.bl[2]), "+v"(f.bl[3]));
}
__device__ __forceinline__ void w4_settle(floatx16 (&acc)[4][4]) {
    asm volatile("s_nop 15\n\ts_nop 15\n\ts_nop 15\n\ts_nop 15\n\ts_nop 15"
                 : "+a"(acc[0][0]), "+a"(acc[0][1]), "+a"(acc[0][2]), "+a"(acc[0][3]), "+a"(acc[1][0]), "+a"(acc[1][1]), "+a"(acc[1][2]), "+a"(acc[1][3]),
                   "+a"(acc[2][0]), "+a"(acc[2][1]), "+a"(acc[2][2]), "+a"(acc[2][3]), "+a"(acc[3][0]), "+a"(acc[3][1]), "+a"(acc[3][2]), "+a"(acc[3][3]));
}
template <int LOFF, bool NT> __device__ __forceinline__ void w4_piece(const char* sbase, unsigned voff, unsigned lds_buf) {
    if constexpr (NT)
        asm volatile("s_add_u32 m0, %2, %3\n\ts_nop 0\n\tglobal_load_lds_dwordx4 %0, %1 nt" : : "v"(voff), "s"(sbase), "s"(lds_buf), "n"(LOFF) : "memory", "scc");
    else
        asm volatile("s_add_u32 m0, %2, %3\n\ts_nop 0\n\tglobal_load_lds_dwordx4 %0, %1" : : "v"(voff), "s"(sbase), "s"(lds_buf), "n"(LOFF) : "memory", "scc");
}

template <class G, int NODMA, bool A_NT>
__device__ __forceinline__ void w4_kloop(const unsigned short* A, int lda, size_t a_plane, const unsigned short* W, int ldw, size_t w_plane,
                                         int M, int N, int K, int m0, int n0, unsigned char* smem, int wave, int wr, int wc, int lane,
                                         floatx16 (&acc)[4][4]) {
    const int hh = lane >> 5, idx = lane & 31;
    unsigned va[G::TA], vw[G::TW];
    {
        const int prow = lane >> 2;
        const unsigned chunkb = (unsigned)(((lane & 3) ^ ((prow >> 2) & 3)) * 16);
#pragma unroll
        for (int t = 0; t < G::TA; ++t) {
            int row = m0 + 16 * (wave + 4 * t) + prow;
            row = row < M ? row : M - 1;
            va[t] = (unsigned)row * (unsigned)lda * 2u + chunkb;
        }
#pragma unroll
        for (int t = 0; t < G::TW; ++t) {
            int col = n0 + 16 * (wave + 4 * t) + prow;
            col = col < N ? col : N - 1;
            vw[t] = (unsigned)col * (unsigned)ldw * 2u + chunkb;
        }
    }
    const char* const a_hi = reinterpret_cast<const char*>(A);
    const char* const a_lo = a_hi + a_plane * 2;
    const char* const w_hi = reinterpret_cast<const char*>(W);
    const char* const w_lo = w_hi + w_plane * 2;
    const unsigned lds0 = __builtin_amdgcn_readfirstlane(lds_addr_of(smem));
    const unsigned ldsw = lds0 + (unsigned)wave * 1024;
    auto piece = [&](auto I, int js, unsigned buf) {
        constexpr int i = decltype(I)::value;
        if constexpr (NODMA == 1) return;
        const size_t ko = (size_t)js * 64;
        if constexpr (i < G::TA) w4_piece<4096 * i, A_NT>(a_hi + ko, va[i], buf);
        else if constexpr (i < 2 * G::TA) w4_piece<G::A_PLANE_B + 4096 * (i - G::TA), A_NT>(a_lo + ko, va[i - G::TA], buf);
        else if constexpr (i < 2 * G::TA + G::TW) w4_piece<2 * G::A_PLANE_B + 4096 * (i - 2 * G::TA), false>(w_hi + ko, vw[i - 2 * G::TA], buf);
        else w4_piece<2 * G::A_PLANE_B + G::W_PLANE_B + 4096 * (i - 2 * G::TA - G::TW), false>(w_lo + ko, vw[i - 2 * G::TA - G::TW], buf);
    };

    const unsigned fsw = (unsigned)((idx >> 2) & 3);
    const unsigned fa0 = lds0 + (unsigned)((wr * 128 + idx) * 64);
    const unsigned fb0 = lds0 + 2 * G::A_PLANE_B + (unsigned)((wc * 128 + idx) * 64);
    auto frag_read = [&](auto Rr, W4Frags& f, unsigned fa, unsigned fb) {
        constexpr int r = decltype(Rr)::value;
        if constexpr (r < 4) w4_read<G::A_PLANE_B + (r & 3) * 2048>(f.al[r & 3], fa);
        else if constexpr (r < 8) w4_read<(r & 3) * 2048>(f.bh[r & 3], fb);
        else if constexpr (r < 12) w4_read<(r & 3) * 2048>(f.ah[r & 3], fa);
        else w4_read<G::W_PLANE_B + (r & 3) * 2048>(f.bl[r & 3], fb);
    };
    auto coff = [&](int st) { return (unsigned)(((2 * st + hh) ^ fsw) * 16); };

    const int ns = K / 32;

    [&]<int... I>(std::integer_sequence<int, I...>) { (piece(std::integral_constant<int, I>{}, 0, ldsw), ...); }(std::make_integer_sequence<int, G::NPW>{});
    if constexpr (NODMA == 0) glds_wait_all();
    __builtin_amdgcn_s_barrier();
    W4Frags f0, f1;
    [&]<int... I>(std::integer_sequence<int, I...>) { (frag_read(std::integral_constant<int, I>{}, f0, fa0 + coff(0), fb0 + coff(0)), ...); }(std::make_integer_sequence<int, 16>{});
    [&]<int... I>(std::integer_sequence<int, I...>) { (piece(std::integral_constant<int, I>{}, 1, ldsw + G::STAGE_B), ...); }(std::make_integer_sequence<int, G::NPW>{});
    w4_reads_done(f0);

#pragma unroll
    for (int i = 0; i < 4; ++i)
#pragma unroll
        for (int j = 0; j < 4; ++j)
#pragma unroll
            for (int r = 0; r < 16; ++r) acc[i][j][r] = 0.f;
    w4_settle(acc);

    auto kstep = [&](auto Issue, W4Frags& x, W4Frags& y, unsigned fa, unsigned fb, int js, unsigned buf) {
        constexpr bool ISSUE = decltype(Issue)::value;
        [&]<int... Gp>(std::integer_sequence<int, Gp...>) {
            ([&] {
                constexpr int g = Gp, P = g >> 4, t = g & 15, i = t >> 2, j = t & 3;
                if constexpr (P == 0) w4_mfma(acc[i][j], x.al[i], x.bh[j]);
                else if constexpr (P == 1) w4_mfma(acc[i][j], x.ah[i], x.bl[j]);
                else w4_mfma(acc[i][j], x.ah[i], x.bh[j]);
                if constexpr ((g & 1) == 0 && g < 32) frag_read(std::integral_constant<int, (g >> 1)>{}, y, fa, fb);
                if constexpr (ISSUE && g >= 1) {
                    constexpr int q = ((g - 1) * G::NPW + 47) / 48;
                    if constexpr (q < G::NPW && (48 * q) / G::NPW + 1 == g) piece(std::integral_constant<int, q>{}, js, buf);
                }
            }(), ...);
        }(std::make_integer_sequence<int, 48>{});
        w4_reads_done(y);
    };
    auto stage = [&](auto Issue, int j) {
        const unsigned cur = (unsigned)(j & 1) * G::STAGE_B, nxt = G::STAGE_B - cur;
        kstep(std::false_type{}, f0, f1, fa0 + cur + coff(1), fb0 + cur + coff(1), 0, 0u);
        if constexpr (NODMA == 0) glds_wait_all();
        __builtin_amdgcn_s_barrier();
        kstep(Issue, f1, f0, fa0 + nxt + coff(0), fb0 + nxt + coff(0), j + 2, ldsw + cur);
    };
    for (int j = 0; j < ns - 2; ++j) stage(std::true_type{}, j);
    stage(std::false_type{}, ns - 2);
    stage(std::false_type{}, ns - 1);
    w4_settle(acc);
}

template <int MODE, int OUT, int EABL, int NODMA>
__global__ __launch_bounds__(256, 1) void gemm_f16x2_w4_kernel(Gemm2Args p, int nM, int nN) {
    typedef W4Geo<2, 2> G;
    extern __shared__ __attribute__((aligned(16))) unsigned char smem[];
    const int L = blockIdx.x;
    const int xcd = L & 7, j8 = L >> 3;
    const int mblk = (j8 / nN) * 8 + xcd, nblk = j8 % nN;
    if (mblk >= nM) return;
    const int m0 = mblk * G::BM, n0 = nblk * G::BN;
    const int lane = threadIdx.x & 63;
    const int wave = __builtin_amdgcn_readfirstlane(threadIdx.x >> 6);
    const int wr = wave >> 1, wc = wave & 1;
    floatx16 acc[4][4];
    w4_kloop<G, NODMA, false>(p.A, p.lda, p.a_plane, p.W, p.ldw, p.w_plane, p.M, p.N, p.K, m0, n0, smem, wave, wr, wc, lane, acc);
    gemm2_epilogue<4, 4, 4, MODE, OUT, EABL>(p, acc, smem, m0, n0, nblk, wave, wr, wc, lane);
}

#if defined(PF_MEASUREMENT_KERNELS)
template <int MODE, bool LN, bool A_NT>
__global__ __launch_bounds__(256, 1) void gemm_f16x2_w4_row_kernel(GemmRowArgs p) {
    typedef W4Geo<1, 4> G;
    static_assert(G::LDS_B == RW_LDS_B && G::BM == RW_BM && G::BN == RW_BN, "the row epilogue's LDS plan");
    extern __shared__ __attribute__((aligned(16))) unsigned char smem[];
    const int m0 = blockIdx.x * G::BM;
    const int tid = threadIdx.x;
    const int lane = tid & 63;
    const int wave = __builtin_amdgcn_readfirstlane(tid >> 6);
    floatx16 acc[4][4];
    w4_kloop<G, 0, A_NT>(p.A, p.lda, p.a_plane, p.W, p.ldw, p.w_plane, p.M, G::BN, p.K, m0, 0, smem, wave, 0, wave, lane, acc);
    gemm2_row_epilogue<MODE, LN, 256, 4, 0>(p, acc, smem, m0, tid, wave, 0, wave, lane, true);
    gemm2_row_epilogue<MODE, LN, 256, 4, 2>(p, acc, smem, m0, tid, wave, 1, wave, lane, false);
}

#endif

template <int MODE, int OUT, int EABL = 0, int NODMA = 0>
int launch_w4(const Gemm2Args& a, hipStream_t stream) {
    typedef W4Geo<2, 2> G;
    static PerDeviceOnce configured;
    if (!configured.done()) {
        PF_HIP_TRY(hipFuncSetAttribute(reinterpret_cast<const void*>(&gemm_f16x2_w4_kernel<MODE, OUT, EABL, NODMA>),
                                       hipFuncAttributeMaxDynamicSharedMemorySize, G::LDS_B));
        configured.mark();
    }
    const int nM = ceil_div(a.M, G::BM), nN = ceil_div(a.N, G::BN);
    const int nMpad = (nM + 7) / 8 * 8;
    hipLaunchKernelGGL((gemm_f16x2_w4_kernel<MODE, OUT, EABL, NODMA>), dim3((unsigned)nMpad * nN), dim3(256), G::LDS_B, stream, a, nM, nN);
    PF_HIP_TRY(hipGetLastError());
    return 0;
}

#if defined(PF_MEASUREMENT_KERNELS)
template <int MODE, bool LN, bool A_NT>
int launch_w4_row_t(const GemmRowArgs& a, hipStream_t stream) {
    typedef W4Geo<1, 4> G;
    static PerDeviceOnce configured;
    if (!configured.done()) {
        PF_HIP_TRY(hipFuncSetAttribute(reinterpret_cast<const void*>(&gemm_f16x2_w4_row_kernel<MODE, LN, A_NT>),
                                       hipFuncAttributeMaxDynamicSharedMemorySize, G::LDS_B));
        configured.mark();
    }
    hipLaunchKernelGGL((gemm_f16x2_w4_row_kernel<MODE, LN, A_NT>), dim3((unsigned)ceil_div(a.M, G::BM)), dim3(256), G::LDS_B, stream, a);
    PF_HIP_TRY(hipGetLastError());
    return 0;
}
template <int MODE, bool LN>
int launch_w4_row_m(const GemmRowArgs& a, hipStream_t stream) {
    return (a.a_nt & 1) ? launch_w4_row_t<MODE, LN, true>(a, stream) : launch_w4_row_t<MODE, LN, false>(a, stream);
}

#endif

}

bool gemm_f16x2_w4_ok(const Gemm2Args& a) {
    return a.K % 32 == 0 && a.K >= 64 && a.N % 256 == 0 && a.kslices <= 1 && a.ksplit <= 1 && !a.amax_val && a.a_kstep <= 0 && a.w_kstep <= 0 &&
           (size_t)a.M * (size_t)a.lda * 2 < (1ull << 32) && (size_t)a.N * (size_t)a.ldw * 2 < (1ull << 32);
}

int launch_gemm_f16x2_w4(const Gemm2Args& a, int abl, hipStream_t stream) {
    PF_REQUIRE(gemm_f16x2_w4_ok(a), "gemm_f16x2 (four-wave shape): needs K % 32 == 0, K >= 64, N % 256 == 0 and operands below 4 GB");
    const int mode = (a.R1 ? 1 : 0) | (a.R2 ? 2 : 0);
    if (a.qkv_D > 0) return launch_w4<0, 2>(a, stream);
    if (a.C2) {
        PF_REQUIRE(mode == 0, "gemm_f16x2: the plane output has no residual form");
#if defined(PF_MEASUREMENT_KERNELS)
        if (abl == 1) return launch_w4<0, 1, 1>(a, stream);
#endif
        return launch_w4<0, 1>(a, stream);
    }
#if defined(PF_MEASUREMENT_KERNELS)
    if (abl == 1) return launch_w4<0, 0, 1>(a, stream);
    if (abl == 2) return launch_w4<0, 0, 2>(a, stream);
    if (abl == 3) return launch_w4<0, 0, 2, 1>(a, stream);
#else
    PF_REQUIRE(abl == 0, "gemm_f16x2 (four-wave shape): the ablation builds are in the measurement library (make measure)");
#endif
    switch (mode) {
        case 0: return launch_w4<0, 0>(a, stream);
        case 1: return launch_w4<1, 0>(a, stream);
        case 2: return launch_w4<2, 0>(a, stream);
        default: return launch_w4<3, 0>(a, stream);
    }
}

bool gemm_f16x2_w4_row_ok(const GemmRowArgs& a) {
    return a.N == 512 && a.K % 32 == 0 && a.K >= 64 && (size_t)a.M * (size_t)a.lda * 2 < (1ull << 32) && (size_t)a.ldw * 1024 < (1ull << 32);
}

#if defined(PF_MEASUREMENT_KERNELS)
int launch_gemm_f16x2_w4_row(const GemmRowArgs& a, hipStream_t stream) {
    PF_REQUIRE(gemm_f16x2_w4_row_ok(a), "gemm_f16x2_row (four-wave shape): needs N == 512, K % 32 == 0, K >= 64 and operands below 4 GB");
    const bool ln = a.ln_g != nullptr;
    if (a.fs_v) return a.R2 ? launch_w4_row_m<6, true>(a, stream) : launch_w4_row_m<4, true>(a, stream);
    const int mode = (a.R1 ? 1 : 0) | (a.R2 ? 2 : 0);
    switch (mode * 2 + (ln ? 1 : 0)) {
        case 0: return launch_w4_row_m<0, false>(a, stream);
        case 1: return launch_w4_row_m<0, true>(a, stream);
        case 2: return launch_w4_row_m<1, false>(a, stream);
        case 3: return launch_w4_row_m<1, true>(a, stream);
        case 4: return launch_w4_row_m<2, false>(a, stream);
        case 5: return launch_w4_row_m<2, true>(a, stream);
        case 6: return launch_w4_row_m<3, false>(a, stream);
        default: return launch_w4_row_m<3, true>(a, stream);
    }
}

#else
int launch_gemm_f16x2_w4_row(const GemmRowArgs&, hipStream_t) {
    set_error("gemm_f16x2_row (four-wave shape): measured and off -- in the measurement library only (make measure)");
    return -1;
}
#endif

}
```

Measured before the change: 38440.

## Switch f16x2 GEMM kernels from 32x32x16 to 16x16x32 MFMA tiles

Replaces the 32x32x16 MFMA instruction with 16x16x32 across the generic, row and four-wave f16x2 GEMM k-loops. Accumulators become floatx4 arrays and the LDS swizzle and fragment offsets are re-derived for the 16-lane layout. The product/read/prefetch schedule is interleaved per column phase, and the epilogues gain a matching 16x16 store and argmax path. It also routes QKV outputs away from the four-wave kernel and confines the ps path to measurement builds. The intent is better issue density or lower register pressure per MFMA. The cost is more instructions and more LDS fragment reads, plus a changed swizzle that could add bank conflicts.

```diff
diff --git a/funasr_amd/csrc/gemm_f16x2.hip b/funasr_amd/csrc/gemm_f16x2.hip
--- a/funasr_amd/csrc/gemm_f16x2.hip
+++ b/funasr_amd/csrc/gemm_f16x2.hip
@@ -40,7 +40,7 @@
     const unsigned short* src[PPW];
     {
         const int prow = lane / CPR;
-        const int chunk = (lane % CPR) ^ ((prow >> G::SWZ) & (CPR - 1));
+        const int chunk = (lane % CPR) ^ ((KS == 32 ? 0 - (prow >> 2) : (prow >> G::SWZ)) & (CPR - 1));
 #pragma unroll
         for (int i = 0; i < PPW; ++i) {
             const int q = wave + G::NW * i;
@@ -63,13 +63,15 @@
         glds16(src[i] + kt * (i < G::A_PIECES / G::NW ? a_step : w_step), lds0 + (unsigned)buf * STAGE_B + (unsigned)i * (G::NW * 1024));
     };
 
-    floatx16 acc[WM][WN];
-#pragma unroll
-    for (int i = 0; i < WM; ++i)
-#pragma unroll
-        for (int jj = 0; jj < WN; ++jj)
-#pragma unroll
-            for (int r = 0; r < 16; ++r) acc[i][jj][r] = 0.f;
+    constexpr bool S16 = KS_ == 32;
+    constexpr int AM = S16 ? 2 * WM : WM, AN = S16 ? 2 * WN : WN, AR = S16 ? 4 : 16;
+    typename std::conditional<S16, floatx4, floatx16>::type acc[AM][AN];
+#pragma unroll
+    for (int i = 0; i < AM; ++i)
+#pragma unroll
+        for (int jj = 0; jj < AN; ++jj)
+#pragma unroll
+            for (int r = 0; r < AR; ++r) acc[i][jj][r] = 0.f;
 
     const int f = (idx >> G::SWZ) & (CPR - 1);
     const int aoff = (wr * (WM * 32) + idx) * ROWB;
@@ -196,6 +198,12 @@
 #undef PF_PROD16
         }
     } else {
+    static_assert(CPR == 4 && G::SWZ == 2, "64-B LDS rows");
+    constexpr int NPH = WN, NG = 3 * NPH;
+    const int q16 = lane >> 4, l16 = lane & 15;
+    const int coff16 = (q16 ^ ((0 - (l16 >> 2)) & 3)) * 16;
+    const int aoff16 = (wr * (WM * 32) + l16) * ROWB + coff16;
+    const int boff16 = 2 * A_PLANE_B + (wc * (WN * 32) + l16) * ROWB + coff16;
 #pragma unroll
     for (int i = 0; i < PPW; ++i) piece(i, 0, 0);
     for (int kt = 0; kt < nk; ++kt) {
@@ -204,52 +212,36 @@
         const bool nxt = kt + 1 < nk;
         const int nb = (kt + 1) & 1;
         const unsigned char* sb = smem + (kt & 1) * STAGE_B;
-#define PF_PIECE(I) do { if ((I) < PPW && nxt) piece((I) < PPW ? (I) : 0, nb, kt + 1); } while (0)
-#define PF_PROD(PA, PB)                                                                                               \
-    _Pragma("unroll") for (int i = 0; i < WM; ++i) _Pragma("unroll") for (int jj = 0; jj < WN; ++jj)                  \
-        acc[i][jj] = __builtin_amdgcn_mfma_f32_32x32x16_f16(a[i][PA], b[jj][PB], acc[i][jj], 0, 0, 0)
-#define PF_LOAD(S)                                                                                                    \
-    _Pragma("unroll") for (int pl = 0; pl < 2; ++pl) {                                                                \
-        _Pragma("unroll") for (int i = 0; i < WM; ++i)                                                                \
-            a[i][pl] = __builtin_bit_cast(f16x8, *reinterpret_cast<const uint4*>(sb + pl * A_PLANE_B + aoff + i * 32 * ROWB + coff[S]));   \
-        _Pragma("unroll") for (int jj = 0; jj < WN; ++jj)                                                             \
-            b[jj][pl] = __builtin_bit_cast(f16x8, *reinterpret_cast<const uint4*>(sb + pl * B_PLANE_B + boff + jj * 32 * ROWB + coff[S])); \
-    }
-        if constexpr (SCHED == 0 || SCHED == 3) {
-            f16x8 a[WM][2], b[WN][2];
-            PF_LOAD(0)
-            PF_PROD(1, 0); PF_PIECE(0); PF_PIECE(1);
-            PF_PROD(0, 1); PF_PIECE(2); PF_PIECE(3);
-            PF_PROD(0, 0); PF_PIECE(4);
-            PF_LOAD(1)
-            PF_PROD(1, 0); PF_PIECE(5); PF_PIECE(6);
-            PF_PROD(0, 1); PF_PIECE(7);
-            PF_PROD(0, 0);
-        } else {
-            f16x8 a[WM][2], b[WN][2], a1[WM][2], b1[WN][2];
-            PF_LOAD(0)
-            {
-#define a a1
-#define b b1
-                PF_LOAD(1)
-#undef a
-#undef b
-            }
-            if constexpr (SCHED == 2) { PF_PIECE(0); PF_PIECE(1); PF_PIECE(2); PF_PIECE(3); }
-            PF_PROD(1, 0); if constexpr (SCHED == 1) { PF_PIECE(0); PF_PIECE(1); } else { PF_PIECE(4); PF_PIECE(5); }
-            PF_PROD(0, 1); if constexpr (SCHED == 1) { PF_PIECE(2); PF_PIECE(3); } else { PF_PIECE(6); PF_PIECE(7); }
-            PF_PROD(0, 0); if constexpr (SCHED == 1) { PF_PIECE(4); }
-#define a a1
-#define b b1
-            PF_PROD(1, 0); if constexpr (SCHED == 1) { PF_PIECE(5); PF_PIECE(6); }
-            PF_PROD(0, 1); if constexpr (SCHED == 1) { PF_PIECE(7); }
-            PF_PROD(0, 0);
-#undef a
-#undef b
-        }
-#undef PF_PROD
-#undef PF_LOAD
-#undef PF_PIECE
+        f16x8 a[2 * WM][2];
+#pragma unroll
+        for (int pl = 1; pl >= 0; --pl)
+#pragma unroll
+            for (int i = 0; i < 2 * WM; ++i)
+                a[i][pl] = __builtin_bit_cast(f16x8, *reinterpret_cast<const uint4*>(sb + pl * A_PLANE_B + aoff16 + i * 16 * ROWB));
+#pragma unroll
+        for (int ph = 0; ph < NPH; ++ph) {
+            f16x8 b[2][2];
+#pragma unroll
+            for (int pl = 0; pl < 2; ++pl)
+#pragma unroll
+                for (int jj = 0; jj < 2; ++jj)
+                    b[jj][pl] = __builtin_bit_cast(f16x8, *reinterpret_cast<const uint4*>(sb + pl * B_PLANE_B + boff16 + (2 * ph + jj) * 16 * ROWB));
+#pragma unroll
+            for (int pr = 0; pr < 3; ++pr) {
+                const int PA = pr == 0 ? 1 : 0, PB = pr == 1 ? 1 : 0;
+#pragma unroll
+                for (int i = 0; i < 2 * WM; ++i)
+#pragma unroll
+                    for (int jj = 0; jj < 2; ++jj)
+                        acc[i][2 * ph + jj] = __builtin_amdgcn_mfma_f32_16x16x32_f16(a[i][PA], b[jj][PB], acc[i][2 * ph + jj], 0, 0, 0);
+                const int g = 3 * ph + pr;
+                if (g < NG - 1 && nxt) {
+#pragma unroll
+                    for (int i = 0; i < PPW; ++i)
+                        if (i >= g * PPW / (NG - 1) && i < (g + 1) * PPW / (NG - 1)) piece(i, nb, kt + 1);
+                }
+            }
+        }
     }
     }
 
@@ -491,6 +483,10 @@
 }
 
 static bool qkv_form_prefers_ps(const Gemm2Args& a) {
+#if !defined(PF_MEASUREMENT_KERNELS)
+    (void)a;
+    return false;
+#endif
     static const int mode = [] { const char* e = getenv("PF_QKV_PS"); return e ? atoi(e) : 2; }();
     if (mode == 0 || !gemm_f16x2_ps_ok(a)) return false;
     if (mode == 1) return true;
@@ -558,7 +554,9 @@
                    "gemm_f16x2: QKV outputs");
     }
     if ((a.tile & 15) == 10 || (a.tile & 15) == 12) {
+#if defined(PF_MEASUREMENT_KERNELS)
         if (gemm_f16x2_ps_ok(a)) return launch_gemm_f16x2_ps(a, stream);
+#endif
         Gemm2Args b = a;
         b.tile = 0;
         return launch_gemm_f16x2(b, stream);
diff --git a/funasr_amd/csrc/gemm_f16x2_epilogue.h b/funasr_amd/csrc/gemm_f16x2_epilogue.h
--- a/funasr_amd/csrc/gemm_f16x2_epilogue.h
+++ b/funasr_amd/csrc/gemm_f16x2_epilogue.h
@@ -3,23 +3,64 @@
 
 namespace pf {
 
-template <int WM, int WN, int NW, int MODE, int OUT, int ABL>
-__device__ __forceinline__ void gemm2_epilogue(const Gemm2Args& p, floatx16 (&acc)[WM][WN], unsigned char* smem, int m0, int n0, int nblk,
+template <int WM, int WN, int NW, int MODE, int OUT, int ABL, typename AT, int AM, int AN>
+__device__ __forceinline__ void gemm2_epilogue(const Gemm2Args& p, AT (&acc)[AM][AN], unsigned char* smem, int m0, int n0, int nblk,
                                                int wave, int wr, int wc, int lane) {
+    constexpr bool S16 = AM == 2 * WM;
+    static_assert((S16 && AN == 2 * WN && sizeof(AT) == 16) || (!S16 && AM == WM && AN == WN && sizeof(AT) == 64), "accumulator tiles");
+    constexpr int AR = S16 ? 4 : 16;
     const int hh = lane >> 5, idx = lane & 31;
+    const int q16 = lane >> 4, l16 = lane & 15;
     constexpr int ELD_ = WN * 32 + 4;
     if constexpr (ABL == 2) {
         float t = 0.f;
 #pragma unroll
-        for (int i = 0; i < WM; ++i)
-#pragma unroll
-            for (int jj = 0; jj < WN; ++jj)
-#pragma unroll
-                for (int r = 0; r < 16; ++r) t += acc[i][jj][r];
+        for (int i = 0; i < AM; ++i)
+#pragma unroll
+            for (int jj = 0; jj < AN; ++jj)
+#pragma unroll
+                for (int r = 0; r < AR; ++r) t += acc[i][jj][r];
         if (t == 123.456f) p.C[0] = t;
         return;
     }
-    if constexpr (OUT == 3) {
+    if constexpr (OUT == 3 && S16) {
+        const float osc = p.oscale_dev ? p.oscale * *p.oscale_dev : p.oscale;
+        float bv[AN];
+#pragma unroll
+        for (int jj = 0; jj < AN; ++jj) {
+            const int col = n0 + wc * (WN * 32) + jj * 16 + l16;
+            bv[jj] = (p.bias && col < p.N) ? p.bias[col] : 0.f;
+        }
+#pragma unroll
+        for (int i = 0; i < AM; ++i) {
+#pragma unroll
+            for (int r = 0; r < 4; ++r) {
+                const int row = m0 + wr * (WM * 32) + i * 16 + 4 * q16 + r;
+                float best = -INFINITY;
+                int besti = 0x7fffffff;
+#pragma unroll
+                for (int jj = 0; jj < AN; ++jj) {
+                    const int col = n0 + wc * (WN * 32) + jj * 16 + l16;
+                    if (col < p.N) {
+                        const float v = acc[i][jj][r] * osc + bv[jj];
+                        if (v > best) { best = v; besti = col; }
+                    }
+                }
+#pragma unroll
+                for (int o = 8; o > 0; o >>= 1) {
+                    const float ov = __shfl_xor(best, o, 64);
+                    const int oi = __shfl_xor(besti, o, 64);
+                    if (ov > best || (ov == best && oi < besti)) { best = ov; besti = oi; }
+                }
+                if (l16 == 0 && row < p.M) {
+                    const size_t o = (size_t)row * p.amax_ld + 2 * nblk + wc;
+                    p.amax_val[o] = best;
+                    p.amax_idx[o] = besti;
+                }
+            }
+        }
+        return;
+    } else if constexpr (OUT == 3) {
         const float osc = p.oscale_dev ? p.oscale * *p.oscale_dev : p.oscale;
         float bv[WN];
 #pragma unroll
@@ -64,6 +105,8 @@
     constexpr int NPASS = 32 / RPS;
     __syncthreads();
     float* slab = reinterpret_cast<float*>(smem) + wave * (32 * ELD);
+    int sw16 = 4 * q16 * ELD + l16;
+    asm volatile("" : "+v"(sw16));
     const int c4 = lane % LPR, rsub = lane / LPR;
     const int col = n0 + wc * (WN * 32) + c4 * 4;
     const bool colok = col + 3 < p.N;
@@ -73,11 +116,21 @@
     if (p.bias && colok) bias4 = *reinterpret_cast<const float4*>(p.bias + col);
 #pragma unroll
     for (int i = 0; i < WM; ++i) {
-#pragma unroll
-        for (int jj = 0; jj < WN; ++jj)
-#pragma unroll
-            for (int r = 0; r < 16; ++r)
-                slab[((r & 3) + 8 * (r >> 2) + 4 * hh) * ELD + jj * 32 + idx] = acc[i][jj][r];
+        if constexpr (S16) {
+#pragma unroll
+            for (int si = 0; si < 2; ++si)
+#pragma unroll
+                for (int jj = 0; jj < AN; ++jj)
+#pragma unroll
+                    for (int r = 0; r < 4; ++r)
+                        slab[sw16 + (si * 16 + r) * ELD + jj * 16] = acc[2 * i + si][jj][r];
+        } else {
+#pragma unroll
+            for (int jj = 0; jj < WN; ++jj)
+#pragma unroll
+                for (int r = 0; r < 16; ++r)
+                    slab[((r & 3) + 8 * (r >> 2) + 4 * hh) * ELD + jj * 32 + idx] = acc[i][jj][r];
+        }
         const int row0 = m0 + wr * (WM * 32) + i * 32 + rsub;
         if (!colok) continue;
         const int seg = OUT == 2 ? n0 / p.qkv_D + (p.kv_form ? 1 : 0) : 0;
diff --git a/funasr_amd/csrc/gemm_f16x2_row.hip b/funasr_amd/csrc/gemm_f16x2_row.hip
--- a/funasr_amd/csrc/gemm_f16x2_row.hip
+++ b/funasr_amd/csrc/gemm_f16x2_row.hip
@@ -23,7 +23,7 @@
     const unsigned short* src[RW_PPW];
     {
         const int prow = lane >> 2;
-        const int chunk = (lane & 3) ^ ((prow >> 2) & 3);
+        const int chunk = (lane & 3) ^ ((0 - (prow >> 2)) & 3);
         int row = m0 + wave * 16 + prow;
         row = row < p.M ? row : p.M - 1;
         src[0] = p.A + (size_t)row * p.lda + chunk * 8;
@@ -42,20 +42,18 @@
         else glds16(src[i] + kt * RW_KS, dst);
     };
 
-    floatx16 acc[WM][WN];
-#pragma unroll
-    for (int i = 0; i < WM; ++i)
-#pragma unroll
-        for (int jj = 0; jj < WN; ++jj)
-#pragma unroll
-            for (int r = 0; r < 16; ++r) acc[i][jj][r] = 0.f;
-
-    const int f = (idx >> 2) & 3;
-    const int aoff = (wr * 64 + idx) * RW_ROWB;
-    const int boff = 2 * RW_A_PLANE_B + (wc * 128 + idx) * RW_ROWB;
-    int coff[2];
-#pragma unroll
-    for (int st = 0; st < 2; ++st) coff[st] = ((2 * st + hh) ^ f) * 16;
+    floatx4 acc[2 * WM][2 * WN];
+#pragma unroll
+    for (int i = 0; i < 2 * WM; ++i)
+#pragma unroll
+        for (int jj = 0; jj < 2 * WN; ++jj)
+#pragma unroll
+            for (int r = 0; r < 4; ++r) acc[i][jj][r] = 0.f;
+
+    const int q16 = lane >> 4, l16 = lane & 15;
+    const int coff16 = (q16 ^ ((0 - (l16 >> 2)) & 3)) * 16;
+    const int aoff = (wr * 64 + l16) * RW_ROWB + coff16;
+    const int boff = 2 * RW_A_PLANE_B + (wc * 128 + l16) * RW_ROWB + coff16;
 
 #if defined(PF_MEASUREMENT_KERNELS)
     const int nk = (p.a_nt & 128) ? 0 : p.K / RW_KS;
@@ -109,41 +107,32 @@
 #else
         constexpr bool early = false;
 #endif
-#define RW_PIECE(I) do { if (nxt && !early) piece(I, nb, kt + 1); } while (0)
-#define RW_PROD(AF, BF, PA, PB)                                                                                       \
-    _Pragma("unroll") for (int i = 0; i < WM; ++i) _Pragma("unroll") for (int jj = 0; jj < WN; ++jj)                  \
-        acc[i][jj] = __builtin_amdgcn_mfma_f32_32x32x16_f16(AF[i][PA], BF[jj][PB], acc[i][jj], 0, 0, 0)
-#define RW_LOAD(AF, BF, S)                                                                                            \
-    _Pragma("unroll") for (int pl = 0; pl < 2; ++pl) {                                                                \
-        _Pragma("unroll") for (int i = 0; i < WM; ++i)                                                                \
-            AF[i][pl] = __builtin_bit_cast(f16x8, *reinterpret_cast<const uint4*>(sb + pl * RW_A_PLANE_B + aoff + i * 32 * RW_ROWB + coff[S]));   \
-        _Pragma("unroll") for (int jj = 0; jj < WN; ++jj)                                                             \
-            BF[jj][pl] = __builtin_bit_cast(f16x8, *reinterpret_cast<const uint4*>(sb + pl * RW_B_PLANE_B + boff + jj * 32 * RW_ROWB + coff[S])); \
-    }
-        f16x8 a0[WM][2], b0[WN][2], a1[WM][2], b1[WN][2];
-        if constexpr (SCHED == 2) {
-            RW_LOAD(a0, b0, 0)
-            RW_LOAD(a1, b1, 1)
-            RW_PIECE(0); RW_PIECE(1); RW_PIECE(2); RW_PIECE(3);
-            RW_PROD(a0, b0, 1, 0); RW_PIECE(4); RW_PIECE(5);
-            RW_PROD(a0, b0, 0, 1); RW_PIECE(6); RW_PIECE(7);
-            RW_PROD(a0, b0, 0, 0); RW_PIECE(8); RW_PIECE(9);
-            RW_PROD(a1, b1, 1, 0);
-            RW_PROD(a1, b1, 0, 1);
-            RW_PROD(a1, b1, 0, 0);
-        } else {
-            RW_LOAD(a0, b0, 0)
-            RW_PROD(a0, b0, 1, 0); RW_PIECE(0); RW_PIECE(1); RW_PIECE(2);
-            RW_PROD(a0, b0, 0, 1); RW_PIECE(3); RW_PIECE(4); RW_PIECE(5);
-            RW_PROD(a0, b0, 0, 0); RW_PIECE(6); RW_PIECE(7);
-            RW_LOAD(a1, b1, 1)
-            RW_PROD(a1, b1, 1, 0); RW_PIECE(8); RW_PIECE(9);
-            RW_PROD(a1, b1, 0, 1);
-            RW_PROD(a1, b1, 0, 0);
-        }
-#undef RW_PROD
-#undef RW_LOAD
-#undef RW_PIECE
+        f16x8 a[2 * WM][2];
+#pragma unroll
+        for (int pl = 1; pl >= 0; --pl)
+#pragma unroll
+            for (int i = 0; i < 2 * WM; ++i)
+                a[i][pl] = __builtin_bit_cast(f16x8, *reinterpret_cast<const uint4*>(sb + pl * RW_A_PLANE_B + aoff + i * 16 * RW_ROWB));
+#pragma unroll
+        for (int ph = 0; ph < WN; ++ph) {
+            f16x8 b[2][2];
+#pragma unroll
+            for (int pl = 0; pl < 2; ++pl)
+#pragma unroll
+                for (int jj = 0; jj < 2; ++jj)
+                    b[jj][pl] = __builtin_bit_cast(f16x8, *reinterpret_cast<const uint4*>(sb + pl * RW_B_PLANE_B + boff + (2 * ph + jj) * 16 * RW_ROWB));
+#pragma unroll
+            for (int pr = 0; pr < 3; ++pr) {
+                const int PA = pr == 0 ? 1 : 0, PB = pr == 1 ? 1 : 0;
+#pragma unroll
+                for (int i = 0; i < 2 * WM; ++i)
+#pragma unroll
+                    for (int jj = 0; jj < 2; ++jj)
+                        acc[i][2 * ph + jj] = __builtin_amdgcn_mfma_f32_16x16x32_f16(a[i][PA], b[jj][PB], acc[i][2 * ph + jj], 0, 0, 0);
+                const int g = 3 * ph + pr;
+                if (g < RW_PPW && nxt && !early) piece(g, nb, kt + 1);
+            }
+        }
     }
 #if defined(PF_MEASUREMENT_KERNELS)
     if (p.a_nt & 256) {
@@ -153,7 +142,7 @@
 #pragma unroll
             for (int jj = 0; jj < WN; ++jj)
 #pragma unroll
-                for (int r = 0; r < 16; ++r) sacc += acc[i][jj][r];
+                for (int r = 0; r < 16; ++r) sacc += acc[2 * i + (r >> 3)][2 * jj + ((r >> 2) & 1)][r & 3];
         if (sacc == 12345.678f && p.C) p.C[tid] = sacc;
         return;
     }
diff --git a/funasr_amd/csrc/gemm_f16x2_row8.hip b/funasr_amd/csrc/gemm_f16x2_row8.hip
--- a/funasr_amd/csrc/gemm_f16x2_row8.hip
+++ b/funasr_amd/csrc/gemm_f16x2_row8.hip
@@ -43,7 +43,7 @@
     const unsigned short* src_w[8];
     {
         const int prow = lane >> 2;
-        const int chunk = (lane & 3) ^ ((prow >> 2) & 3);
+        const int chunk = (lane & 3) ^ ((0 - (prow >> 2)) & 3);
 #pragma unroll
         for (int j = 0; j < 2; ++j) {
             const int a = (wave + 8 * j) < NA ? wave + 8 * j : wave;
@@ -68,20 +68,18 @@
         glds16(src_w[j] + kt * R8_KS, lds0 + (unsigned)buf * STAGE_B + 2 * A_PLANE_B + (unsigned)(wave + 8 * j) * 1024);
     };
 
-    floatx16 acc[WM][2];
-#pragma unroll
-    for (int i = 0; i < WM; ++i)
-#pragma unroll
-        for (int jj = 0; jj < 2; ++jj)
-#pragma unroll
-            for (int r = 0; r < 16; ++r) acc[i][jj][r] = 0.f;
-
-    const int f = (idx >> 2) & 3;
-    const int aoff = idx * R8_ROWB;
-    const int boff = 2 * A_PLANE_B + (wave * 64 + idx) * R8_ROWB;
-    int coff[2];
-#pragma unroll
-    for (int st = 0; st < 2; ++st) coff[st] = ((2 * st + hh) ^ f) * 16;
+    floatx4 acc[2 * WM][4];
+#pragma unroll
+    for (int i = 0; i < 2 * WM; ++i)
+#pragma unroll
+        for (int jj = 0; jj < 4; ++jj)
+#pragma unroll
+            for (int r = 0; r < 4; ++r) acc[i][jj][r] = 0.f;
+
+    const int q16 = lane >> 4, l16 = lane & 15;
+    const int coff16 = (q16 ^ ((0 - (l16 >> 2)) & 3)) * 16;
+    const int aoff = l16 * R8_ROWB + coff16;
+    const int boff = 2 * A_PLANE_B + (wave * 64 + l16) * R8_ROWB + coff16;
 
     const int nk = p.K / R8_KS;
     piece_a(0, 0, 0);
@@ -94,28 +92,25 @@
         const bool nxt = kt + 1 < nk;
         const int nb = (kt + 1) & 1;
         const unsigned char* sb = smem + (kt & 1) * STAGE_B;
-#define R8_PROD(AF, BF, PA, PB)                                                                                       \
-    _Pragma("unroll") for (int i = 0; i < WM; ++i) _Pragma("unroll") for (int jj = 0; jj < 2; ++jj)                   \
-        acc[i][jj] = __builtin_amdgcn_mfma_f32_32x32x16_f16(AF[i][PA], BF[jj][PB], acc[i][jj], 0, 0, 0)
-#define R8_LOAD(AF, BF, S)                                                                                            \
-    _Pragma("unroll") for (int pl = 0; pl < 2; ++pl) {                                                                \
-        _Pragma("unroll") for (int i = 0; i < WM; ++i)                                                                \
-            AF[i][pl] = __builtin_bit_cast(f16x8, *reinterpret_cast<const uint4*>(sb + pl * A_PLANE_B + aoff + i * 32 * R8_ROWB + coff[S]));     \
-        _Pragma("unroll") for (int jj = 0; jj < 2; ++jj)                                                              \
-            BF[jj][pl] = __builtin_bit_cast(f16x8, *reinterpret_cast<const uint4*>(sb + pl * R8_B_PLANE_B + boff + jj * 32 * R8_ROWB + coff[S])); \
-    }
-        f16x8 a0[WM][2], b0[2][2], a1[WM][2], b1[2][2];
-        R8_LOAD(a0, b0, 0)
-        R8_LOAD(a1, b1, 1)
+#define R8_PROD(PA, PB)                                                                                               \
+    _Pragma("unroll") for (int i = 0; i < 2 * WM; ++i) _Pragma("unroll") for (int jj = 0; jj < 4; ++jj)               \
+        acc[i][jj] = __builtin_amdgcn_mfma_f32_16x16x32_f16(a[i][PA], b[jj][PB], acc[i][jj], 0, 0, 0)
+        f16x8 a[2 * WM][2], b[4][2];
+#pragma unroll
+        for (int pl = 1; pl >= 0; --pl)
+#pragma unroll
+            for (int i = 0; i < 2 * WM; ++i)
+                a[i][pl] = __builtin_bit_cast(f16x8, *reinterpret_cast<const uint4*>(sb + pl * A_PLANE_B + aoff + i * 16 * R8_ROWB));
+#pragma unroll
+        for (int pl = 0; pl < 2; ++pl)
+#pragma unroll
+            for (int jj = 0; jj < 4; ++jj)
+                b[jj][pl] = __builtin_bit_cast(f16x8, *reinterpret_cast<const uint4*>(sb + pl * R8_B_PLANE_B + boff + jj * 16 * R8_ROWB));
         if (nxt) { piece_a(0, nb, kt + 1); if (has_a1) piece_a(1, nb, kt + 1); piece_w(0, nb, kt + 1); piece_w(1, nb, kt + 1); }
-        R8_PROD(a0, b0, 1, 0); if (nxt) { piece_w(2, nb, kt + 1); piece_w(3, nb, kt + 1); }
-        R8_PROD(a0, b0, 0, 1); if (nxt) { piece_w(4, nb, kt + 1); piece_w(5, nb, kt + 1); }
-        R8_PROD(a0, b0, 0, 0); if (nxt) { piece_w(6, nb, kt + 1); piece_w(7, nb, kt + 1); }
-        R8_PROD(a1, b1, 1, 0);
-        R8_PROD(a1, b1, 0, 1);
-        R8_PROD(a1, b1, 0, 0);
+        R8_PROD(1, 0); if (nxt) { piece_w(2, nb, kt + 1); piece_w(3, nb, kt + 1); piece_w(4, nb, kt + 1); }
+        R8_PROD(0, 1); if (nxt) { piece_w(5, nb, kt + 1); piece_w(6, nb, kt + 1); piece_w(7, nb, kt + 1); }
+        R8_PROD(0, 0);
 #undef R8_PROD
-#undef R8_LOAD
     }
 
     constexpr bool HAS_R1 = (MODE & 1) != 0, HAS_R2 = (MODE & 2) != 0, FSMN = (MODE & 4) != 0;
@@ -129,6 +124,8 @@
     float4 bias4 = make_float4(0.f, 0.f, 0.f, 0.f);
     if (p.bias) bias4 = *reinterpret_cast<const float4*>(p.bias + col);
     float4 ov[WM][8];
+    int sw16 = 4 * q16 * R8_ELD + q * 64 + l16;
+    asm volatile("" : "+v"(sw16));
 #pragma unroll
     for (int i = 0; i < WM; ++i) {
         __syncthreads();
@@ -140,10 +137,12 @@
             }
         }
 #pragma unroll
-        for (int jj = 0; jj < 2; ++jj)
-#pragma unroll
-            for (int r = 0; r < 16; ++r)
-                slab[((r & 3) + 8 * (r >> 2) + 4 * hh) * R8_ELD + q * 64 + jj * 32 + idx] = acc[i][jj][r];
+        for (int si = 0; si < 2; ++si)
+#pragma unroll
+            for (int jj = 0; jj < 4; ++jj)
+#pragma unroll
+                for (int r = 0; r < 4; ++r)
+                    slab[sw16 + (si * 16 + r) * R8_ELD + jj * 16] = acc[2 * i + si][jj][r];
         __syncthreads();
         const int rl0 = q * 16 + rsub * 8;
         const int row0 = m0 + i * 32 + rl0;
diff --git a/funasr_amd/csrc/gemm_f16x2_row_epilogue.h b/funasr_amd/csrc/gemm_f16x2_row_epilogue.h
--- a/funasr_amd/csrc/gemm_f16x2_row_epilogue.h
+++ b/funasr_amd/csrc/gemm_f16x2_row_epilogue.h
@@ -17,12 +17,16 @@
 static_assert(RW_SLAB_B <= RW_LDS_B && (RW_P_FLOATS + 2 * RW_BM) * 4 <= RW_LDS_B, "epilogue LDS");
 static_assert(RW_FSW_OFF_B + RW_FS_KS * RW_BN * 4 <= RW_LDS_B, "FSMN taps do not fit behind the slabs");
 
-template <int MODE, bool LN, int NT, int AM, int I0>
-__device__ __forceinline__ void gemm2_row_epilogue(const GemmRowArgs& p, floatx16 (&accf)[AM][4], unsigned char* smem, int m0, int tid,
+template <int MODE, bool LN, int NT, int AM, int I0, typename AT, int AM_, int AN_>
+__device__ __forceinline__ void gemm2_row_epilogue(const GemmRowArgs& p, AT (&accf)[AM_][AN_], unsigned char* smem, int m0, int tid,
                                                    int wave, int wr, int wc, int lane, bool stage_taps) {
     constexpr int WM = 2, WN = 4;
+    constexpr bool S16 = AN_ == 8;
+    static_assert((S16 && AM_ == 2 * AM && sizeof(AT) == 16) || (!S16 && AM_ == AM && AN_ == 4 && sizeof(AT) == 64), "accumulator tiles");
     const int hh = lane >> 5, idx = lane & 31;
-    floatx16 (&acc_)[AM][4] = accf;
+    int sw16 = 4 * (lane >> 4) * RW_ELD + (lane & 15);
+    asm volatile("" : "+v"(sw16));
+    AT (&acc_)[AM_][AN_] = accf;
 #if defined(PF_MEASUREMENT_KERNELS)
     const int abl = p.a_nt;
 #else
@@ -53,11 +57,21 @@
     float4 ov[WM][16];
 #pragma unroll
     for (int i = 0; i < WM; ++i) {
-#pragma unroll
-        for (int jj = 0; jj < WN; ++jj)
-#pragma unroll
-            for (int r = 0; r < 16; ++r)
-                slab[((r & 3) + 8 * (r >> 2) + 4 * hh) * RW_ELD + jj * 32 + idx] = acc(i, jj)[r];
+        if constexpr (S16) {
+#pragma unroll
+            for (int si = 0; si < 2; ++si)
+#pragma unroll
+                for (int jj = 0; jj < 8; ++jj)
+#pragma unroll
+                    for (int r = 0; r < 4; ++r)
+                        slab[sw16 + (si * 16 + r) * RW_ELD + jj * 16] = acc_[2 * (I0 + i) + si][jj][r];
+        } else {
+#pragma unroll
+            for (int jj = 0; jj < WN; ++jj)
+#pragma unroll
+                for (int r = 0; r < 16; ++r)
+                    slab[((r & 3) + 8 * (r >> 2) + 4 * hh) * RW_ELD + jj * 32 + idx] = acc(i, jj)[r];
+        }
         const int row0 = m0 + wr * 64 + i * 32 + rsub * 16;
         if constexpr (FSMN) {
             const int grp = row0 >> 4;
diff --git a/funasr_amd/csrc/gemm_f16x2_w4.hip b/funasr_amd/csrc/gemm_f16x2_w4.hip
--- a/funasr_amd/csrc/gemm_f16x2_w4.hip
+++ b/funasr_amd/csrc/gemm_f16x2_w4.hip
@@ -19,23 +19,26 @@
     static_assert(GM * GN == 4 && NPW == 2 * (TA + TW), "four waves");
 };
 
-struct W4Frags { f16x8 al[4], ah[4], bh[4], bl[4]; };
-
-__device__ __forceinline__ void w4_mfma(floatx16& acc, const f16x8& a, const f16x8& b) {
-    asm volatile("v_mfma_f32_32x32x16_f16 %0, %1, %2, %0" : "+a"(acc) : "v"(a), "v"(b));
+struct W4Frags { f16x8 al[8], ah[8], bl[8], bh[8]; };
+
+__device__ __forceinline__ void w4_mfma(floatx4& acc, const f16x8& a, const f16x8& b) {
+    asm volatile("v_mfma_f32_16x16x32_f16 %0, %1, %2, %0" : "+a"(acc) : "v"(a), "v"(b));
 }
 template <int OFF> __device__ __forceinline__ void w4_read(f16x8& dst, unsigned addr) {
     asm volatile("ds_read_b128 %0, %1 offset:%2" : "=v"(dst) : "v"(addr), "n"(OFF));
 }
+__device__ __forceinline__ void w4_tie8(f16x8 (&x)[8]) {
+    asm volatile("" : "+v"(x[0]), "+v"(x[1]), "+v"(x[2]), "+v"(x[3]), "+v"(x[4]), "+v"(x[5]), "+v"(x[6]), "+v"(x[7]));
+}
 __device__ __forceinline__ void w4_reads_done(W4Frags& f) {
-    asm volatile("s_waitcnt lgkmcnt(0)"
-                 : "+v"(f.al[0]), "+v"(f.al[1]), "+v"(f.al[2]), "+v"(f.al[3]), "+v"(f.ah[0]), "+v"(f.ah[1]), "+v"(f.ah[2]), "+v"(f.ah[3]),
-                   "+v"(f.bh[0]), "+v"(f.bh[1]), "+v"(f.bh[2]), "+v"(f.bh[3]), "+v"(f.bl[0]), "+v"(f.bl[1]), "+v"(f.bl[2]), "+v"(f.bl[3]));
-}
-__device__ __forceinline__ void w4_settle(floatx16 (&acc)[4][4]) {
-    asm volatile("s_nop 15\n\ts_nop 15\n\ts_nop 15\n\ts_nop 15\n\ts_nop 15"
-                 : "+a"(acc[0][0]), "+a"(acc[0][1]), "+a"(acc[0][2]), "+a"(acc[0][3]), "+a"(acc[1][0]), "+a"(acc[1][1]), "+a"(acc[1][2]), "+a"(acc[1][3]),
-                   "+a"(acc[2][0]), "+a"(acc[2][1]), "+a"(acc[2][2]), "+a"(acc[2][3]), "+a"(acc[3][0]), "+a"(acc[3][1]), "+a"(acc[3][2]), "+a"(acc[3][3]));
+    asm volatile("s_waitcnt lgkmcnt(0)" ::: "memory");
+    w4_tie8(f.al); w4_tie8(f.ah); w4_tie8(f.bl); w4_tie8(f.bh);
+}
+__device__ __forceinline__ void w4_settle(floatx4 (&acc)[8][8]) {
+    asm volatile("s_nop 15\n\ts_nop 15\n\ts_nop 15\n\ts_nop 15\n\ts_nop 15" ::: "memory");
+#pragma unroll
+    for (int i = 0; i < 8; ++i)
+        asm volatile("" : "+a"(acc[i][0]), "+a"(acc[i][1]), "+a"(acc[i][2]), "+a"(acc[i][3]), "+a"(acc[i][4]), "+a"(acc[i][5]), "+a"(acc[i][6]), "+a"(acc[i][7]));
 }
 template <int LOFF, bool NT> __device__ __forceinline__ void w4_piece(const char* sbase, unsigned voff, unsigned lds_buf) {
     if constexpr (NT)
@@ -47,12 +50,12 @@
 template <class G, int NODMA, bool A_NT>
 __device__ __forceinline__ void w4_kloop(const unsigned short* A, int lda, size_t a_plane, const unsigned short* W, int ldw, size_t w_plane,
                                          int M, int N, int K, int m0, int n0, unsigned char* smem, int wave, int wr, int wc, int lane,
-                                         floatx16 (&acc)[4][4]) {
-    const int hh = lane >> 5, idx = lane & 31;
+                                         floatx4 (&acc)[8][8]) {
+    const int q16 = lane >> 4, l16 = lane & 15;
     unsigned va[G::TA], vw[G::TW];
     {
         const int prow = lane >> 2;
-        const unsigned chunkb = (unsigned)(((lane & 3) ^ ((prow >> 2) & 3)) * 16);
+        const unsigned chunkb = (unsigned)(((lane & 3) ^ ((0 - (prow >> 2)) & 3)) * 16);
 #pragma unroll
         for (int t = 0; t < G::TA; ++t) {
             int row = m0 + 16 * (wave + 4 * t) + prow;
@@ -82,59 +85,65 @@
         else w4_piece<2 * G::A_PLANE_B + G::W_PLANE_B + 4096 * (i - 2 * G::TA - G::TW), false>(w_lo + ko, vw[i - 2 * G::TA - G::TW], buf);
     };
 
-    const unsigned fsw = (unsigned)((idx >> 2) & 3);
-    const unsigned fa0 = lds0 + (unsigned)((wr * 128 + idx) * 64);
-    const unsigned fb0 = lds0 + 2 * G::A_PLANE_B + (unsigned)((wc * 128 + idx) * 64);
-    auto frag_read = [&](auto Rr, W4Frags& f, unsigned fa, unsigned fb) {
-        constexpr int r = decltype(Rr)::value;
-        if constexpr (r < 4) w4_read<G::A_PLANE_B + (r & 3) * 2048>(f.al[r & 3], fa);
-        else if constexpr (r < 8) w4_read<(r & 3) * 2048>(f.bh[r & 3], fb);
-        else if constexpr (r < 12) w4_read<(r & 3) * 2048>(f.ah[r & 3], fa);
-        else w4_read<G::W_PLANE_B + (r & 3) * 2048>(f.bl[r & 3], fb);
-    };
-    auto coff = [&](int st) { return (unsigned)(((2 * st + hh) ^ fsw) * 16); };
+    const unsigned coff16 = (unsigned)((q16 ^ ((0 - (l16 >> 2)) & 3)) * 16);
+    const unsigned fa0 = lds0 + (unsigned)((wr * 128 + l16) * 64) + coff16;
+    const unsigned fb0 = lds0 + 2 * G::A_PLANE_B + (unsigned)((wc * 128 + l16) * 64) + coff16;
 
     const int ns = K / 32;
 
     [&]<int... I>(std::integer_sequence<int, I...>) { (piece(std::integral_constant<int, I>{}, 0, ldsw), ...); }(std::make_integer_sequence<int, G::NPW>{});
     if constexpr (NODMA == 0) glds_wait_all();
     __builtin_amdgcn_s_barrier();
-    W4Frags f0, f1;
-    [&]<int... I>(std::integer_sequence<int, I...>) { (frag_read(std::integral_constant<int, I>{}, f0, fa0 + coff(0), fb0 + coff(0)), ...); }(std::make_integer_sequence<int, 16>{});
+    W4Frags f;
+    [&]<int... T>(std::integer_sequence<int, T...>) { (w4_read<G::A_PLANE_B + T * 1024>(f.al[T], fa0), ...); }(std::make_integer_sequence<int, 8>{});
+    [&]<int... T>(std::integer_sequence<int, T...>) { (w4_read<T * 1024>(f.bh[T], fb0), ...); }(std::make_integer_sequence<int, 8>{});
     [&]<int... I>(std::integer_sequence<int, I...>) { (piece(std::integral_constant<int, I>{}, 1, ldsw + G::STAGE_B), ...); }(std::make_integer_sequence<int, G::NPW>{});
-    w4_reads_done(f0);
-
-#pragma unroll
-    for (int i = 0; i < 4; ++i)
-#pragma unroll
-        for (int j = 0; j < 4; ++j)
-#pragma unroll
-            for (int r = 0; r < 16; ++r) acc[i][j][r] = 0.f;
+    w4_reads_done(f);
+
+#pragma unroll
+    for (int i = 0; i < 8; ++i)
+#pragma unroll
+        for (int j = 0; j < 8; ++j)
+#pragma unroll
+            for (int r = 0; r < 4; ++r) acc[i][j][r] = 0.f;
     w4_settle(acc);
 
-    auto kstep = [&](auto Issue, W4Frags& x, W4Frags& y, unsigned fa, unsigned fb, int js, unsigned buf) {
+    auto product = [&](auto Ph, auto Issue, unsigned fa, unsigned fb, int js, unsigned buf) {
+        constexpr int PH = decltype(Ph)::value;
         constexpr bool ISSUE = decltype(Issue)::value;
         [&]<int... Gp>(std::integer_sequence<int, Gp...>) {
             ([&] {
-                constexpr int g = Gp, P = g >> 4, t = g & 15, i = t >> 2, j = t & 3;
-                if constexpr (P == 0) w4_mfma(acc[i][j], x.al[i], x.bh[j]);
-                else if constexpr (P == 1) w4_mfma(acc[i][j], x.ah[i], x.bl[j]);
-                else w4_mfma(acc[i][j], x.ah[i], x.bh[j]);
-                if constexpr ((g & 1) == 0 && g < 32) frag_read(std::integral_constant<int, (g >> 1)>{}, y, fa, fb);
-                if constexpr (ISSUE && g >= 1) {
-                    constexpr int q = ((g - 1) * G::NPW + 47) / 48;
-                    if constexpr (q < G::NPW && (48 * q) / G::NPW + 1 == g) piece(std::integral_constant<int, q>{}, js, buf);
+                constexpr int g = Gp, i = PH == 2 ? (g & 7) : (g >> 3), j = PH == 2 ? (g >> 3) : (g & 7);
+                if constexpr (PH == 0) w4_mfma(acc[i][j], f.al[i], f.bh[j]);
+                else if constexpr (PH == 1) w4_mfma(acc[i][j], f.ah[i], f.bl[j]);
+                else w4_mfma(acc[i][j], f.ah[i], f.bh[j]);
+                if constexpr (PH == 0 && (g & 3) == 0) {
+                    constexpr int r = g >> 2;
+                    if constexpr (r < 8) w4_read<r * 1024>(f.ah[r], fa);
+                    else w4_read<G::W_PLANE_B + (r - 8) * 1024>(f.bl[r - 8], fb);
+                }
+                if constexpr (PH == 1 && (g & 7) == 0) w4_read<G::A_PLANE_B + (g >> 3) * 1024>(f.al[g >> 3], fa);
+                if constexpr (PH == 2 && (g & 7) == 0 && g >= 8) w4_read<((g >> 3) - 1) * 1024>(f.bh[(g >> 3) - 1], fb);
+                if constexpr (ISSUE && PH == 1 && g >= 1) {
+                    constexpr int q = ((g - 1) * G::NPW + 63) / 64;
+                    if constexpr (q < G::NPW && (64 * q) / G::NPW + 1 == g) piece(std::integral_constant<int, q>{}, js, buf);
                 }
             }(), ...);
-        }(std::make_integer_sequence<int, 48>{});
-        w4_reads_done(y);
+        }(std::make_integer_sequence<int, 64>{});
+        if constexpr (PH == 2) w4_read<7 * 1024>(f.bh[7], fb);
     };
+    typedef std::integral_constant<int, 0> I0;
+    typedef std::integral_constant<int, 1> I1;
+    typedef std::integral_constant<int, 2> I2;
     auto stage = [&](auto Issue, int j) {
         const unsigned cur = (unsigned)(j & 1) * G::STAGE_B, nxt = G::STAGE_B - cur;
-        kstep(std::false_type{}, f0, f1, fa0 + cur + coff(1), fb0 + cur + coff(1), 0, 0u);
+        product(I0{}, std::false_type{}, fa0 + cur, fb0 + cur, 0, 0u);
+        w4_reads_done(f);
         if constexpr (NODMA == 0) glds_wait_all();
         __builtin_amdgcn_s_barrier();
-        kstep(Issue, f1, f0, fa0 + nxt + coff(0), fb0 + nxt + coff(0), j + 2, ldsw + cur);
+        product(I1{}, Issue, fa0 + nxt, fb0 + nxt, j + 2, ldsw + cur);
+        product(I2{}, Issue, fa0 + nxt, fb0 + nxt, j + 2, ldsw + cur);
+        w4_reads_done(f);
     };
     for (int j = 0; j < ns - 2; ++j) stage(std::true_type{}, j);
     stage(std::false_type{}, ns - 2);
@@ -154,7 +163,7 @@
     const int lane = threadIdx.x & 63;
     const int wave = __builtin_amdgcn_readfirstlane(threadIdx.x >> 6);
     const int wr = wave >> 1, wc = wave & 1;
-    floatx16 acc[4][4];
+    floatx4 acc[8][8];
     w4_kloop<G, NODMA, false>(p.A, p.lda, p.a_plane, p.W, p.ldw, p.w_plane, p.M, p.N, p.K, m0, n0, smem, wave, wr, wc, lane, acc);
     gemm2_epilogue<4, 4, 4, MODE, OUT, EABL>(p, acc, smem, m0, n0, nblk, wave, wr, wc, lane);
 }
@@ -169,7 +178,7 @@
     const int tid = threadIdx.x;
     const int lane = tid & 63;
     const int wave = __builtin_amdgcn_readfirstlane(tid >> 6);
-    floatx16 acc[4][4];
+    floatx4 acc[8][8];
     w4_kloop<G, 0, A_NT>(p.A, p.lda, p.a_plane, p.W, p.ldw, p.w_plane, p.M, G::BN, p.K, m0, 0, smem, wave, 0, wave, lane, acc);
     gemm2_row_epilogue<MODE, LN, 256, 4, 0>(p, acc, smem, m0, tid, wave, 0, wave, lane, true);
     gemm2_row_epilogue<MODE, LN, 256, 4, 2>(p, acc, smem, m0, tid, wave, 1, wave, lane, false);
@@ -217,14 +226,13 @@
 }
 
 bool gemm_f16x2_w4_ok(const Gemm2Args& a) {
-    return a.K % 32 == 0 && a.K >= 64 && a.N % 256 == 0 && a.kslices <= 1 && a.ksplit <= 1 && !a.amax_val && a.a_kstep <= 0 && a.w_kstep <= 0 &&
+    return a.qkv_D <= 0 && a.K % 32 == 0 && a.K >= 64 && a.N % 256 == 0 && a.kslices <= 1 && a.ksplit <= 1 && !a.amax_val && a.a_kstep <= 0 && a.w_kstep <= 0 &&
            (size_t)a.M * (size_t)a.lda * 2 < (1ull << 32) && (size_t)a.N * (size_t)a.ldw * 2 < (1ull << 32);
 }
 
 int launch_gemm_f16x2_w4(const Gemm2Args& a, int abl, hipStream_t stream) {
     PF_REQUIRE(gemm_f16x2_w4_ok(a), "gemm_f16x2 (four-wave shape): needs K % 32 == 0, K >= 64, N % 256 == 0 and operands below 4 GB");
     const int mode = (a.R1 ? 1 : 0) | (a.R2 ? 2 : 0);
-    if (a.qkv_D > 0) return launch_w4<0, 2>(a, stream);
     if (a.C2) {
         PF_REQUIRE(mode == 0, "gemm_f16x2: the plane output has no residual form");
 #if defined(PF_MEASUREMENT_KERNELS)
```

Measured after the change: 40430, median of 6. +5.2%, better.
